# lpylpy0514/VitTracker

Hardware: AMD Instinct MI355X
Metric: track() frames/sec per GPU, vit_48_h32, 128px search / 64px template (higher is better)
Workload: dtype f32

## Files before the change

### vittracker_amd/csrc/vt_bf3.h

```cpp
#pragma once
#include "vt_common.h"

namespace vt3 {

typedef __bf16 bf16x8 __attribute__((ext_vector_type(8)));
typedef unsigned u32x2 __attribute__((ext_vector_type(2)));
typedef unsigned u32x4 __attribute__((ext_vector_type(4)));

#ifndef VT_SPLIT_DOT2
#define VT_SPLIT_DOT2 0
#endif
typedef __bf16 bf16x2 __attribute__((ext_vector_type(2)));
__device__ __forceinline__ void sub_pair(unsigned pair, float x0, float x1, float& r0, float& r1) {
    const bf16x2 a = __builtin_bit_cast(bf16x2, pair);
    unsigned sel_lo = 0x0000bf80u, sel_hi = 0xbf800000u;
    asm volatile("" : "+s"(sel_lo), "+s"(sel_hi));
    r0 = __builtin_amdgcn_fdot2_f32_bf16(a, __builtin_bit_cast(bf16x2, sel_lo), x0, false);
    r1 = __builtin_amdgcn_fdot2_f32_bf16(a, __builtin_bit_cast(bf16x2, sel_hi), x1, false);
}
__device__ __forceinline__ void split3(f4 x, u32x2& h, u32x2& m, u32x2& l) {
#ifdef VT_SPLIT_FAKE
    h = u32x2{__builtin_amdgcn_perm(__float_as_uint(x[1]), __float_as_uint(x[0]), 0x07060302u), __builtin_amdgcn_perm(__float_as_uint(x[3]), __float_as_uint(x[2]), 0x07060302u)};
    m = h; l = h;
    asm volatile("" : "+v"(m), "+v"(l));
    return;
#endif
#if VT_SPLIT_DOT2
#pragma unroll
    for (int p = 0; p < 2; ++p) {
        const float x0 = x[2 * p], x1 = x[2 * p + 1];
        float r0, r1, s0, s1;
        h[p] = __builtin_amdgcn_perm(__float_as_uint(x1), __float_as_uint(x0), 0x07060302u);
        sub_pair(h[p], x0, x1, r0, r1);
        m[p] = __builtin_amdgcn_perm(__float_as_uint(r1), __float_as_uint(r0), 0x07060302u);
        sub_pair(m[p], r0, r1, s0, s1);
        l[p] = __builtin_amdgcn_perm(__float_as_uint(s1), __float_as_uint(s0), 0x07060302u);
    }
#else
    unsigned xb[4], r1b[4], r2b[4];
#pragma unroll
    for (int i = 0; i < 4; ++i) {
        xb[i] = __float_as_uint(x[i]);
        const float r1 = x[i] - __uint_as_float(xb[i] & 0xffff0000u);
        r1b[i] = __float_as_uint(r1);
        const float r2 = r1 - __uint_as_float(r1b[i] & 0xffff0000u);
        r2b[i] = __float_as_uint(r2);
    }
    h = u32x2{__builtin_amdgcn_perm(xb[1], xb[0], 0x07060302u), __builtin_amdgcn_perm(xb[3], xb[2], 0x07060302u)};
    m = u32x2{__builtin_amdgcn_perm(r1b[1], r1b[0], 0x07060302u), __builtin_amdgcn_perm(r1b[3], r1b[2], 0x07060302u)};
    l = u32x2{__builtin_amdgcn_perm(r2b[1], r2b[0], 0x07060302u), __builtin_amdgcn_perm(r2b[3], r2b[2], 0x07060302u)};
#endif
}
__device__ __forceinline__ f4 join3(u32x2 h, u32x2 m, u32x2 l) {
    f4 v;
#pragma unroll
    for (int i = 0; i < 4; ++i) {
        const unsigned sh = (i & 1) ? 0u : 16u;
        const float fh = __uint_as_float((h[i >> 1] << sh) & 0xffff0000u), fm = __uint_as_float((m[i >> 1] << sh) & 0xffff0000u),
                    fl = __uint_as_float((l[i >> 1] << sh) & 0xffff0000u);
        v[i] = (fh + fm) + fl;
    }
    return v;
}

__device__ __forceinline__ f4 mma(u32x4 a, u32x4 b, f4 acc) {
    return __builtin_amdgcn_mfma_f32_16x16x32_bf16(__builtin_bit_cast(bf16x8, a), __builtin_bit_cast(bf16x8, b), acc, 0, 0, 0);
}
typedef short s16x4 __attribute__((ext_vector_type(4)));
__device__ __forceinline__ f4 mma16(u32x2 a, u32x2 b, f4 acc) {
    return __builtin_amdgcn_mfma_f32_16x16x16bf16_1k(__builtin_bit_cast(s16x4, a), __builtin_bit_cast(s16x4, b), acc, 0, 0, 0);
}
__device__ __forceinline__ f4 mma_small(const u32x4 (&a)[3], const u32x4 (&b)[3], f4 acc) {
    acc = mma(a[2], b[0], acc);
    acc = mma(a[0], b[2], acc);
    return mma(a[1], b[1], acc);
}
__device__ __forceinline__ f4 mma_large(const u32x4 (&a)[3], const u32x4 (&b)[3], f4 acc) {
    acc = mma(a[1], b[0], acc);
    acc = mma(a[0], b[1], acc);
    return mma(a[0], b[0], acc);
}

}
```

### vittracker_amd/csrc/vt_blocks.h

```cpp
#pragma once
#include <type_traits>
#include "vt_common.h"
#include "vt_bf3.h"

namespace vtb {

constexpr int C = 48;
constexpr int NC = C / 16;
constexpr int HID = 4 * C;
constexpr int NH = HID / 16;
constexpr float LN_EPS = 1e-5f;

constexpr int O_LN1G = 0;
constexpr int O_LN1B = O_LN1G + C;
constexpr int O_WQKV = O_LN1B + C;
constexpr int O_BQKV = O_WQKV + 9 * NC * 256;
constexpr int O_WPROJ = O_BQKV + 3 * C;
constexpr int O_BPROJ = O_WPROJ + NC * NC * 256;
constexpr int O_LN2G = O_BPROJ + C;
constexpr int O_LN2B = O_LN2G + C;
constexpr int O_W1 = O_LN2B + C;
constexpr int O_B1 = O_W1 + NH * NC * 256;
constexpr int O_W2 = O_B1 + HID;
constexpr int O_B2 = O_W2 + NC * NH * 256;
constexpr int BLOCK_STRIDE = O_B2 + C;
static_assert(BLOCK_STRIDE % 4 == 0 && O_WQKV % 4 == 0 && O_W1 % 4 == 0 && O_W2 % 4 == 0, "16B alignment");

constexpr int W3_FC1_TILES = NH * 3 + NH * 3 / 2;
constexpr int W3_FC1_OT16 = 3 * 64 + 3 * 32;
constexpr int W3_FC2_TILES = NC * (NH / 2) * 3;
constexpr int W3_QKV_TILES = (9 * W3_FC1_OT16 + 63) / 64;
constexpr int W3_PROJ_TILES = (NC * W3_FC1_OT16 + 63) / 64;
constexpr int BLOCK3_STRIDE = (W3_FC1_TILES + W3_FC2_TILES + W3_QKV_TILES + W3_PROJ_TILES) * 256;
static_assert(W3_FC1_TILES == 54 && W3_FC2_TILES == 54 && NH * W3_FC1_OT16 == W3_FC1_TILES * 64, "three-piece MLP images");

constexpr int S_LN1G = 0;
constexpr int S_LN1B = S_LN1G + C;
constexpr int S_BQKV = S_LN1B + C;
constexpr int S_BPROJ = S_BQKV + 3 * C;
constexpr int S_LN2G = S_BPROJ + C;
constexpr int S_LN2B = S_LN2G + C;
constexpr int S_B1 = S_LN2B + C;
constexpr int S_B2 = S_B1 + HID;
constexpr int SMALL_STRIDE = S_B2 + C;
static_assert(SMALL_STRIDE % 4 == 0 && S_BQKV % 4 == 0 && S_BPROJ % 4 == 0 && S_B1 % 4 == 0 && S_B2 % 4 == 0, "16B alignment");
static_assert(O_LN1B == O_LN1G + C && O_LN2G == O_BPROJ + C && O_LN2B == O_LN2G + C, "contiguous sections");
__host__ __device__ constexpr int small_floats(int depth) { return depth * SMALL_STRIDE + 2 * C; }

__device__ __forceinline__ size_t small_src(int f, int depth) {
    const int blk = f / SMALL_STRIDE, r = f - blk * SMALL_STRIDE;
    if (blk >= depth) return (size_t)depth * BLOCK_STRIDE + r;
    const int o = r < S_BQKV ? O_LN1G + r : r < S_BPROJ ? O_BQKV + (r - S_BQKV) : r < S_B1 ? O_BPROJ + (r - S_BPROJ)
                : r < S_B2 ? O_B1 + (r - S_B1) : O_B2 + (r - S_B2);
    return (size_t)blk * BLOCK_STRIDE + o;
}

__device__ __forceinline__ f4 wimg(const float* __restrict__ base, int tile, int lane) {
    return ld4(base + (size_t)tile * 256 + lane * 4);
}

__device__ __forceinline__ opnd wimg_o(const opnd* __restrict__ base, int tile, int lane) { return base[(size_t)tile * 64 + lane]; }

template <int N>
__device__ __forceinline__ void wburst(f4 (&a)[N], const float* __restrict__ base, int first, int stride, int lane) {
#pragma unroll
    for (int j = 0; j < N; ++j) a[j] = wimg(base, first + j * stride, lane);
    __builtin_amdgcn_sched_barrier(0);
}

template <int N, int VALU_PER_MFMA>
__device__ __forceinline__ void interleave_mfma_valu() {
#pragma unroll
    for (int n = 0; n < N; ++n) {
        __builtin_amdgcn_sched_group_barrier(0x008, 1, 0);
        __builtin_amdgcn_sched_group_barrier(0x002, VALU_PER_MFMA, 0);
    }
}

template <bool AFFINE = true>
__device__ __forceinline__ void layer_norm_img(const f4 (&x)[NC], f4 (&h)[NC], const float* __restrict__ g,
                                               const float* __restrict__ b, int q) {
    static_assert(NC == 3, "three feature chunks");
    const float mean = quad_sum(hsum4((x[0] + x[1]) + x[2])) * (1.0f / C);
    f4 d[NC];
#pragma unroll
    for (int c = 0; c < NC; ++c) d[c] = x[c] - splat4(mean);
    const f4 v4 = __builtin_elementwise_fma(d[2], d[2], __builtin_elementwise_fma(d[1], d[1], d[0] * d[0]));
    const float inv = __builtin_amdgcn_rsqf(quad_sum(hsum4(v4)) * (1.0f / C) + LN_EPS);
#pragma unroll
    for (int c = 0; c < NC; ++c) {
        if constexpr (AFFINE) {
            const f4 gg = ld4(g + 16 * c + 4 * q), bb = ld4(b + 16 * c + 4 * q);
            h[c] = d[c] * splat4(inv) * gg + bb;
        } else {
            h[c] = d[c] * splat4(inv);
        }
    }
}
__device__ __forceinline__ void layer_norm_plain(const f4 (&x)[NC], f4 (&h)[NC]) { layer_norm_img<false>(x, h, nullptr, nullptr, 0); }

constexpr int WBUF_TILES = NH * NC;
template <bool STAGED>
__device__ __forceinline__ void barrier_publish() {
    if constexpr (STAGED) asm volatile("s_waitcnt vmcnt(0)" ::: "memory");
    __syncthreads();
}

#ifndef VT_BLK_GUESTS
#define VT_BLK_GUESTS 1
#endif
#ifndef VT_BLK_OWNERS
#define VT_BLK_OWNERS 1
#endif
#ifndef VT_BLK_NOSTAGE
#define VT_BLK_NOSTAGE 0
#endif
__device__ __forceinline__ void stage_tiles(f4* dst, const float* __restrict__ src, int ntiles, int w, int nw, int lane, bool first_block = true) {
    if (VT_BLK_NOSTAGE == 1 || (VT_BLK_NOSTAGE == 2 && !first_block)) return;
    for (int t = w; t < ntiles; t += nw)
        __builtin_amdgcn_global_load_lds((const __attribute__((address_space(1))) void*)(src + (size_t)t * 256 + lane * 4),
                                         (__attribute__((address_space(3))) void*)(dst + t * 64), 16, 0, 0);
}

template <int NCHUNK, int N, bool SHARED_IS_B, bool PRELOAD_ALL = true, typename AT = opnd, typename OpA, typename OpS>
__device__ __forceinline__ void gemm_stage(OpA opa, OpS ops, f4 (&acc)[N]) {
    if constexpr (PRELOAD_ALL && NCHUNK * N <= 24) {
        AT a[NCHUNK][N];
#pragma unroll
        for (int c = 0; c < NCHUNK; ++c) opa(c, a[c]);
        __builtin_amdgcn_sched_barrier(0);
#pragma unroll
        for (int c = 0; c < NCHUNK; ++c) {
            if constexpr (SHARED_IS_B) mfma4_shared_b(a[c], ops(c), acc);
            else mfma4_shared_a(ops(c), a[c], acc);
        }
    } else {
        AT a[2][N];
        opa(0, a[0]);
#pragma unroll
        for (int c = 0; c < NCHUNK; ++c) {
            if (c + 1 < NCHUNK) opa(c + 1, a[(c + 1) & 1]);
            if constexpr (SHARED_IS_B) mfma4_shared_b(a[c & 1], ops(c), acc);
            else mfma4_shared_a(ops(c), a[c & 1], acc);
        }
    }
}

template <int NT, int NW, int TPW, bool WLDS, bool BAL = false, bool ZC = false, bool BF3 = false, bool A3 = false>
__global__ __launch_bounds__(NW * 64, (NW == 5 && !WLDS) ? 3 : 1) void blocks_kernel(const float* __restrict__ tokens,
                                                         const float* __restrict__ params,
                                                         float* __restrict__ feat,
                                                         float* __restrict__ resid,
                                                         int len_z, int depth_total, int nblocks,
                                                         int dbg_skip_tile,
                                                         unsigned long long* __restrict__ stamps,
                                                         float* __restrict__ zcache,
                                                         int zcache_mode,
                                                         const float* __restrict__ params3,
                                                         unsigned* __restrict__ vlscr) {
    static_assert(NW * TPW >= NT, "tiles must be covered");
    constexpr bool BF3L = BF3 && WLDS, BF3G = BF3 && !WLDS;
    static_assert(!BF3L || (BAL && 2 * NT * NC >= W3_FC2_TILES - WBUF_TILES), "BF3 with staging: written for the balanced frame form; fc2's third output tile is staged in the K / V area");
    static_assert(!BAL || (WLDS && TPW == 1 && NW == 2 * (NT - 1)), "balanced variant: NT-1 owners + NT-1 guests");
    static_assert(!A3 || BF3, "A3: written for the three-piece forms");
    constexpr bool VP3 = A3 && BF3L;
    constexpr bool VP2L = A3 && BF3G;
    constexpr int KP_T16 = W3_FC1_OT16, VP_PAIRS = NT / 2, VP_T16 = VP_PAIRS * 3 * 64 + (NT & 1) * 3 * 32;
    constexpr int KV_UNITS = A3 ? NT * KP_T16 + (VP3 ? NC * VP_T16 : NC * NT * 64) : 2 * NT * NC * 64;
    constexpr int L = NT * 16;
    constexpr int NOWN = BAL ? NT - 1 : NT;
    const int toff = (BAL && len_z == 16) ? 1 : 0;
    const int GT = toff ? 0 : NT - 1;
    extern __shared__ __attribute__((aligned(16))) float lds[];
    f4* Kimg = reinterpret_cast<f4*>(lds);
    f4* Vimg = Kimg + (A3 ? NT * KP_T16 : NT * NC * 64);
    opnd* const Ko = reinterpret_cast<opnd*>(Kimg);
    opnd* const Vo = reinterpret_cast<opnd*>(Vimg);
    f4* Wa = Kimg + KV_UNITS;
    constexpr int WA_TILES = BF3L ? W3_FC1_TILES : WBUF_TILES;
    f4* Wb = Wa + WA_TILES * 64;
    float* Sp = reinterpret_cast<float*>(WLDS ? Wb + WBUF_TILES * 64 : Wa);
    f4* const Gx = reinterpret_cast<f4*>(Sp + small_floats(depth_total));
    f4* Qg = A3 ? Wb + W3_PROJ_TILES * 64 : Gx;
    f4* Pg = Qg + (A3 ? KP_T16 : NC * 64);
    f4* Dg = A3 ? Gx : Pg + 4 * NC * 64;
    float* Mg = reinterpret_cast<float*>(A3 ? Pg + 4 * NC * 64 : Dg + NC * 64);
    int* gflag = A3 ? reinterpret_cast<int*>(Dg + NC * 64) : reinterpret_cast<int*>(Mg + 4 * 2 * 64);
    f4* Pg2 = A3 ? Wa + W3_QKV_TILES * 64 : Pg;
    static_assert(!A3 || (W3_PROJ_TILES * 64 + KP_T16 + 4 * NC * 64 + 4 * 2 * 64 / 4 <= WBUF_TILES * 64 && W3_QKV_TILES * 64 + 4 * NC * 64 <= W3_FC1_TILES * 64),
                  "A3: the exchange areas fit behind proj's / qkv's image");

    const int b = blockIdx.x;
    const int lane = threadIdx.x & 63;
    const int w = __builtin_amdgcn_readfirstlane(threadIdx.x >> 6);
    const int tok = lane & 15, q = lane >> 4;
    const int g = w - (NT - 1);
    const float scale = 0.14433756729740643f;
    constexpr float SCALE_LOG2E = 0.14433756729740643f * 1.4426950408889634f;
    const int guest_prio = dbg_skip_tile == -3 ? 0 : 1;
    const bool fine = dbg_skip_tile == -2 || dbg_skip_tile <= -100;
    if (dbg_skip_tile <= -100) dbg_skip_tile = -100 - dbg_skip_tile;
    int nstamp = 0;
    auto stamp = [&]() {
        if (stamps != nullptr) {
            unsigned long long t;
            asm volatile("s_memtime %0\n\ts_waitcnt lgkmcnt(0)" : "=s"(t)::"memory");
            if (lane == 0) stamps[((size_t)b * NW + w) * 64 + nstamp] = t;
            ++nstamp;
        }
    };
    auto fstamp = [&]() { if (fine) stamp(); };
    stamp();
    auto stage_img = [&](f4* dst, int off, int ntiles, int blk_of) {
        if constexpr (VT_IS_F16)
            stage_tiles(dst, reinterpret_cast<const float*>(reinterpret_cast<const _Float16*>(params3) + (size_t)blk_of * BLOCK_STRIDE + off), (ntiles + 1) / 2, w, NW, lane);
        else
            stage_tiles(dst, params + (size_t)blk_of * BLOCK_STRIDE + off, ntiles, w, NW, lane);
    };
    if constexpr (BF3L) stage_tiles(Wa, params3 + (W3_FC1_TILES + W3_FC2_TILES) * 256, W3_QKV_TILES, w, NW, lane);
    else if constexpr (WLDS) stage_img(Wa, O_WQKV, 9 * NC, 0);
    for (int i = threadIdx.x; 4 * i < small_floats(depth_total); i += NW * 64)
        st4(Sp + 4 * i, ld4(params + small_src(4 * i, depth_total)));

    f4 x[TPW][NC];
#pragma unroll
    for (int i = 0; i < TPW; ++i) {
        const int T = w + NW * i + toff;
        if (T - toff < NOWN && T != dbg_skip_tile) {
            const float* src = tokens + ((size_t)b * L + 16 * T + tok) * C + 4 * q;
#pragma unroll
            for (int c = 0; c < NC; ++c) x[i][c] = ld4(src + 16 * c);
        }
    }
    f4 x4s[NC];
    f4 (&x4)[NC] = (BAL && !BF3) ? x[0] : x4s;
    if constexpr (BAL) {
        if (w >= NOWN) {
            const float* src = tokens + ((size_t)b * L + 16 * GT + tok) * C + 4 * q;
#pragma unroll
            for (int c = 0; c < NC; ++c) x4[c] = ld4(src + 16 * c);
        }
        if (threadIdx.x == 0) *gflag = 0;
        if (w >= NOWN && guest_prio > 0) __builtin_amdgcn_s_setprio(2);
    }
    barrier_publish<WLDS>();

    const int lane_k = lane;
    for (int blk = 0; blk < nblocks; ++blk) {
        int lane_s = lane_k;
        if constexpr (BF3) asm volatile("" : "+v"(lane_s));
        const int lane = lane_s, tok = lane & 15, q = lane >> 4;
        const bool last_skip_z = (blk == depth_total - 1) && (resid == nullptr);
        const bool guest_skip = BAL && last_skip_z && toff != 0;
        const bool zg_tile = BAL && ZC && blk == 0 && toff != 0;
        const float* __restrict__ P = params + (size_t)blk * BLOCK_STRIDE;
        const float* S = Sp + blk * SMALL_STRIDE;
        const opnd* const Po = VT_IS_F16 ? reinterpret_cast<const opnd*>(reinterpret_cast<const _Float16*>(params3) + (size_t)blk * BLOCK_STRIDE)
                                         : reinterpret_cast<const opnd*>(P);
        const opnd* const Wa_o = reinterpret_cast<const opnd*>(Wa);
        const opnd* const Wb_o = reinterpret_cast<const opnd*>(Wb);
        auto w_qkv = [&](int t) { return WLDS ? Wa_o[t * 64 + lane] : wimg_o(Po + O_WQKV / 4, t, lane); };
        auto w_proj = [&](int t) { return WLDS ? Wb_o[t * 64 + lane] : wimg_o(Po + O_WPROJ / 4, t, lane); };
        auto w_fc1 = [&](int t) { return WLDS ? Wa_o[t * 64 + lane] : wimg_o(Po + O_W1 / 4, t, lane); };
        auto w_fc2 = [&](int t) { return WLDS ? Wb_o[t * 64 + lane] : wimg_o(Po + O_W2 / 4, t, lane); };
        const float* __restrict__ P3 = BF3 ? params3 + (size_t)blk * BLOCK3_STRIDE : nullptr;
        constexpr int PROJ_TILES = NC * NC;
        using vt3::u32x2;
        using vt3::u32x4;
        int lane3 = lane;
        if constexpr (BF3) asm volatile("" : "+v"(lane3));
        const auto Wa3 = BF3L ? lds_lane_base<u32x4>(Wa, 16u * lane3) : nullptr;
        const auto Wa3h = BF3L ? lds_lane_base<u32x2>(Wa, 192u * 16u + 8u * lane3) : nullptr;
        const auto Wb3 = BF3L ? lds_lane_base<u32x4>(Wb, 16u * lane3) : nullptr;
        const auto Wk3 = BF3L ? lds_lane_base<u32x4>(Kimg, 16u * lane3) : nullptr;
        auto w1_load3 = [&](int t, u32x4 (&a0)[3], u32x2 (&a2)[3]) {
#pragma unroll
            for (int pc = 0; pc < 3; ++pc) {
                a0[pc] = Wa3[t * W3_FC1_OT16 + pc * 64];
                a2[pc] = Wa3h[t * W3_FC1_OT16 * 2 + pc * 64];
            }
        };
        auto w2_load3 = [&](int p, u32x4 (&a)[NC][3]) {
#pragma unroll
            for (int ot = 0; ot < NC; ++ot)
#pragma unroll
                for (int pc = 0; pc < 3; ++pc)
                    a[ot][pc] = ot < 2 ? Wb3[((ot * (NH / 2) + p) * 3 + pc) * 64] : Wk3[(p * 3 + pc) * 64];
        };
        auto split_h3 = [&](const f4 (&h)[NC], u32x4 (&hb)[3], u32x2 (&hc)[3]) {
            u32x2 a[3], b2[3];
            vt3::split3(h[0], a[0], a[1], a[2]);
            vt3::split3(h[1], b2[0], b2[1], b2[2]);
            vt3::split3(h[2], hc[0], hc[1], hc[2]);
#pragma unroll
            for (int pc = 0; pc < 3; ++pc) hb[pc] = u32x4{a[pc].x, a[pc].y, b2[pc].x, b2[pc].y};
        };
        auto tile48 = [&](auto swap, const u32x4 (&a0)[3], const u32x2 (&a2)[3], const u32x4 (&hb)[3], const u32x2 (&hc)[3], f4 init) {
            constexpr bool SWAP = decltype(swap)::value;
            constexpr int TW[6] = {2, 0, 1, 1, 0, 0}, TX[6] = {0, 2, 1, 0, 1, 0};
            f4 accA = init, accB = splat4(0.f);
#pragma unroll
            for (int e = 0; e < 6; ++e) {
                accB = SWAP ? vt3::mma16(hc[TX[e]], a2[TW[e]], accB) : vt3::mma16(a2[TW[e]], hc[TX[e]], accB);
                accA = SWAP ? vt3::mma(hb[TX[e]], a0[TW[e]], accA) : vt3::mma(a0[TW[e]], hb[TX[e]], accA);
            }
            return accA + accB;
        };
        const auto Kp3 = A3 ? lds_lane_base<u32x4>(Kimg, 16u * lane3) : nullptr;
        const auto Kp3h = A3 ? lds_lane_base<u32x2>(Kimg, 192u * 16u + 8u * lane3) : nullptr;
        const auto Vp3 = A3 ? lds_lane_base<u32x4>(Kimg + NT * KP_T16, 16u * lane3) : nullptr;
        const auto Vp3h = A3 ? lds_lane_base<u32x2>(Kimg + NT * KP_T16, VP_PAIRS * 3 * 64 * 16u + 8u * lane3) : nullptr;
        auto k_load3 = [&](int J, u32x4 (&a0)[3], u32x2 (&a2)[3]) {
#pragma unroll
            for (int pc = 0; pc < 3; ++pc) {
                a0[pc] = Kp3[J * KP_T16 + pc * 64];
                a2[pc] = Kp3h[J * KP_T16 * 2 + pc * 64];
            }
        };
        auto wp_load3 = [&](int t, u32x4 (&a0)[3], u32x2 (&a2)[3]) {
            if constexpr (BF3L) {
#pragma unroll
                for (int pc = 0; pc < 3; ++pc) {
                    a0[pc] = Wb3[t * W3_FC1_OT16 + pc * 64];
                    a2[pc] = reinterpret_cast<const u32x2*>(Wb)[(t * W3_FC1_OT16 + 192) * 2 + pc * 64 + lane3];
                }
            } else {
                const u32x4* const Gp = reinterpret_cast<const u32x4*>(P3) + (W3_FC1_TILES + W3_FC2_TILES + W3_QKV_TILES) * 64;
#pragma unroll
                for (int pc = 0; pc < 3; ++pc) {
                    a0[pc] = Gp[t * W3_FC1_OT16 + pc * 64 + lane3];
                    a2[pc] = reinterpret_cast<const u32x2*>(Gp)[(t * W3_FC1_OT16 + 192) * 2 + pc * 64 + lane3];
                }
            }
        };
        auto store_k3 = [&](f4* dst_tile, const f4 (&kr)[NC]) {
            u32x4 kb[3];
            u32x2 kc[3];
            split_h3(kr, kb, kc);
#pragma unroll
            for (int pc = 0; pc < 3; ++pc) {
                reinterpret_cast<u32x4*>(dst_tile)[pc * 64 + lane3] = kb[pc];
                reinterpret_cast<u32x2*>(dst_tile + 192)[pc * 64 + lane3] = kc[pc];
            }
        };
        auto store_k3c = [&](f4* dst_tile, int ot, f4 r) {
            u32x2 pk[3];
            vt3::split3(r, pk[0], pk[1], pk[2]);
#pragma unroll
            for (int pc = 0; pc < 3; ++pc) {
                if (ot < 2) reinterpret_cast<u32x2*>(dst_tile)[(pc * 64 + lane3) * 2 + ot] = pk[pc];
                else reinterpret_cast<u32x2*>(dst_tile + 192)[pc * 64 + lane3] = pk[pc];
            }
        };
        auto store_v3 = [&](int T, int ot, f4 r) {
            u32x2 pv[3];
            vt3::split3(r, pv[0], pv[1], pv[2]);
            u32x2* base = reinterpret_cast<u32x2*>(Kimg + NT * KP_T16 + ot * VP_T16);
            if ((NT & 1) && T == NT - 1) {
#pragma unroll
                for (int pc = 0; pc < 3; ++pc) base[VP_PAIRS * 3 * 64 * 2 + pc * 64 + lane3] = pv[pc];
            } else {
#pragma unroll
                for (int pc = 0; pc < 3; ++pc) base[(((T >> 1) * 3 + pc) * 64 + lane3) * 2 + (T & 1)] = pv[pc];
            }
        };
        constexpr int VL_BLK_U4 = NC * VP_PAIRS * 64;
        u32x4* const vl_blk = VP2L ? reinterpret_cast<u32x4*>(vlscr) + ((size_t)b * depth_total + blk) * VL_BLK_U4 : nullptr;
        auto store_v2l = [&](int T, int ot, f4 r) {
            u32x2 pv[3];
            vt3::split3(r, pv[0], pv[1], pv[2]);
            const int pp = T >> 1, hf = T & 1;
#pragma unroll
            for (int pc = 0; pc < 2; ++pc) reinterpret_cast<u32x2*>(Vimg)[((((ot * VP_PAIRS + pp) * 2 + pc) * 64) + lane3) * 2 + hf] = pv[pc];
            reinterpret_cast<u32x2*>(vl_blk)[(((ot * VP_PAIRS + pp) * 64) + lane3) * 2 + hf] = pv[2];
        };
        if constexpr (A3 && BF3L) {
            stage_tiles(Wb, P3 + (W3_FC1_TILES + W3_FC2_TILES + W3_QKV_TILES) * 256, W3_PROJ_TILES, w, NW, lane, blk == 0);
        } else if constexpr (BF3L) {
            stage_tiles(Wb, P + O_WPROJ, PROJ_TILES, w, NW, lane, blk == 0);
        } else if constexpr (WLDS) stage_img(Wb, O_WPROJ, NC * NC, blk);

        f4 qr[TPW][NC];
#pragma unroll
        for (int i = 0; i < TPW; ++i) {
            const int T = w + NW * i + toff;
            const bool z_tile = ZC && blk == 0 && 16 * T < len_z;
            int lane_z = lane;
            if constexpr (ZC) asm volatile("" : "+v"(lane_z));
            f4* const zc = reinterpret_cast<f4*>(zcache) + (((size_t)b * (len_z >> 4) + T) * 3 * NC) * 64 + lane_z;
            if (VT_BLK_OWNERS && T - toff < NOWN && T != dbg_skip_tile && z_tile && zcache_mode == 2) {
#pragma unroll
                for (int ot = 0; ot < NC; ++ot) {
                    qr[i][ot] = zc[ot * 64];
                    if constexpr (VP3) store_v3(T, ot, zc[(2 * NC + ot) * 64]);
                    else if constexpr (VP2L) store_v2l(T, ot, zc[(2 * NC + ot) * 64]);
                    else Vo[(ot * NT + T) * 64 + lane] = to_opnd(zc[(2 * NC + ot) * 64]);
                    if constexpr (!A3) Ko[(T * NC + ot) * 64 + lane] = to_opnd(zc[(NC + ot) * 64]);
                }
                if constexpr (A3) {
                    f4 kr[NC];
#pragma unroll
                    for (int ot = 0; ot < NC; ++ot) kr[ot] = zc[(NC + ot) * 64];
                    store_k3(Kimg + T * KP_T16, kr);
                }
            } else if (VT_BLK_OWNERS && T - toff < NOWN && T != dbg_skip_tile) {
                f4 h[NC];
                layer_norm_plain(x[i], h);
                fstamp();
                if constexpr (BF3) {
                    u32x4 hb[3];
                    u32x2 hc[3];
                    split_h3(h, hb, hc);
                    const u32x4* const Gq = reinterpret_cast<const u32x4*>(P3) + (W3_FC1_TILES + W3_FC2_TILES) * 64;
                    const u32x2* const Gqh = reinterpret_cast<const u32x2*>(Gq);
                    auto wq_load3 = [&](int t, u32x4 (&a0)[3], u32x2 (&a2)[3]) {
                        if constexpr (BF3L) w1_load3(t, a0, a2);
                        else {
#pragma unroll
                            for (int pc = 0; pc < 3; ++pc) {
                                a0[pc] = Gq[t * W3_FC1_OT16 + pc * 64 + lane3];
                                a2[pc] = Gqh[(t * W3_FC1_OT16 + 192) * 2 + pc * 64 + lane3];
                            }
                        }
                    };
                    u32x4 a0[2][3];
                    u32x2 a2[2][3];
                    auto bias_q = [&](int t) { return t < 2 * NC ? ld4(S + S_BQKV + 16 * t + 4 * q) : splat4(S[S_BQKV + 2 * C + 16 * (t % NC) + tok]); };
                    f4 bias[2];
                    f4 kr[NC];
                    wq_load3(0, a0[0], a2[0]);
                    bias[0] = bias_q(0);
#pragma unroll
                    for (int t = 0; t < 3 * NC; ++t) {
                        if (t + 1 < 3 * NC) {
                            wq_load3(t + 1, a0[(t + 1) & 1], a2[(t + 1) & 1]);
                            bias[(t + 1) & 1] = bias_q(t + 1);
                        }
                        const int ot = t % NC;
                        f4 r;
                        __builtin_amdgcn_sched_barrier(0);
                        if (t < 2 * NC) r = tile48(std::false_type{}, a0[t & 1], a2[t & 1], hb, hc, bias[t & 1]);
                        else r = tile48(std::true_type{}, a0[t & 1], a2[t & 1], hb, hc, bias[t & 1]);
                        if (t < NC) qr[i][ot] = r;
                        else if constexpr (A3) {
                            if (t < 2 * NC) {
                                if constexpr (VP3) {
                                    kr[ot] = r;
                                    if (ot == NC - 1) store_k3(Kimg + T * KP_T16, kr);
                                } else store_k3c(Kimg + T * KP_T16, ot, r);
                            } else if constexpr (VP3) store_v3(T, ot, r);
                            else if constexpr (VP2L) store_v2l(T, ot, r);
                            else Vo[(ot * NT + T) * 64 + lane] = to_opnd(r);
                        }
                        else if (t < 2 * NC) Ko[(T * NC + ot) * 64 + lane] = to_opnd(r);
                        else Vo[(ot * NT + T) * 64 + lane] = to_opnd(r);
                        if (z_tile && zcache_mode == 1) zc[t * 64] = r;
                        if (t == 2 * NC - 1) fstamp();
                    }
                } else {
                {
                    f4 acc[2 * NC];
#pragma unroll
                    for (int ot = 0; ot < 2 * NC; ++ot) acc[ot] = ld4(S + S_BQKV + 16 * ot + 4 * q);
                    gemm_stage<NC, 2 * NC, true, WLDS>(
                        [&](int c, opnd (&a)[2 * NC]) {
#pragma unroll
                            for (int ot = 0; ot < 2 * NC; ++ot) a[ot] = w_qkv(ot * NC + c);
                        },
                        [&](int c) { return h[c]; }, acc);
#pragma unroll
                    for (int ot = 0; ot < NC; ++ot) {
                        qr[i][ot] = acc[ot];
                        Ko[(T * NC + ot) * 64 + lane] = to_opnd(acc[NC + ot]);
                        if (z_tile && zcache_mode == 1) { zc[ot * 64] = acc[ot]; zc[(NC + ot) * 64] = acc[NC + ot]; }
                    }
                }
                fstamp();
                {
                    f4 acc[NC];
#pragma unroll
                    for (int ot = 0; ot < NC; ++ot) acc[ot] = splat4(S[S_BQKV + 2 * C + 16 * ot + tok]);
                    gemm_stage<NC, NC, false, WLDS>(
                        [&](int c, opnd (&bw)[NC]) {
#pragma unroll
                            for (int ot = 0; ot < NC; ++ot) bw[ot] = w_qkv((2 * NC + ot) * NC + c);
                        },
                        [&](int c) { return h[c]; }, acc);
#pragma unroll
                    for (int ot = 0; ot < NC; ++ot) {
                        Vo[(ot * NT + T) * 64 + lane] = to_opnd(acc[ot]);
                        if (z_tile && zcache_mode == 1) zc[(2 * NC + ot) * 64] = acc[ot];
                    }
                }
                }
            }
        }
        if constexpr (BAL) {
            auto zc_guest = [&]() {
                int lane_z = lane;
                asm volatile("" : "+v"(lane_z));
                return reinterpret_cast<f4*>(zcache) + ((size_t)b * 3 * NC + NC * g) * 64 + lane_z;
            };
            auto with_gt = [&](auto f) {
                if (toff) f(std::integral_constant<int, 0>{});
                else f(std::integral_constant<int, NT - 1>{});
            };
            const bool guest_qkv = VT_BLK_GUESTS && w >= NOWN && g < 3 && !(guest_skip && g == 0);
            if (BF3L && guest_qkv) {
                f4 r[NC];
                if (zg_tile && zcache_mode == 2) {
                    const f4* const zc = zc_guest();
#pragma unroll
                    for (int j = 0; j < NC; ++j) r[j] = zc[j * 64];
                } else {
                    f4 h[NC];
                    layer_norm_plain(x4, h);
                    u32x4 hb[3];
                    u32x2 hc[3];
                    split_h3(h, hb, hc);
                    u32x4 a0[NC][3];
                    u32x2 a2[NC][3];
#pragma unroll
                    for (int j = 0; j < NC; ++j) w1_load3(NC * g + j, a0[j], a2[j]);
                    if (g < 2) {
                        f4 bias[NC];
#pragma unroll
                        for (int j = 0; j < NC; ++j) bias[j] = ld4(S + S_BQKV + 16 * (g * NC + j) + 4 * q);
                        __builtin_amdgcn_sched_barrier(0);
#pragma unroll
                        for (int j = 0; j < NC; ++j) r[j] = tile48(std::false_type{}, a0[j], a2[j], hb, hc, bias[j]);
                    } else {
                        f4 bias[NC];
#pragma unroll
                        for (int j = 0; j < NC; ++j) bias[j] = splat4(S[S_BQKV + 2 * C + 16 * j + tok]);
                        __builtin_amdgcn_sched_barrier(0);
#pragma unroll
                        for (int j = 0; j < NC; ++j) r[j] = tile48(std::true_type{}, a0[j], a2[j], hb, hc, bias[j]);
                    }
                    if (zg_tile && zcache_mode == 1) {
                        f4* const zc = zc_guest();
#pragma unroll
                        for (int j = 0; j < NC; ++j) zc[j * 64] = r[j];
                    }
                }
                with_gt([&](auto gt) {
                    constexpr int GTc = decltype(gt)::value;
                    if (g < 2) {
                        if constexpr (A3) {
                            store_k3(g == 0 ? Qg : Kimg + GTc * KP_T16, r);
                        } else {
#pragma unroll
                            for (int j = 0; j < NC; ++j) {
                                if (g == 0) Qg[j * 64 + lane] = r[j];
                                else Ko[(GTc * NC + j) * 64 + lane] = to_opnd(r[j]);
                            }
                        }
                    } else {
#pragma unroll
                        for (int j = 0; j < NC; ++j) {
                            if constexpr (A3) store_v3(GTc, j, r[j]);
                            else Vo[(j * NT + GTc) * 64 + lane] = to_opnd(r[j]);
                        }
                    }
                });
            } else if (guest_qkv) {
                f4 acc[NC];
                if (zg_tile && zcache_mode == 2) {
                    const f4* const zc = zc_guest();
#pragma unroll
                    for (int ot = 0; ot < NC; ++ot) acc[ot] = zc[ot * 64];
                } else {
                    f4 h[NC];
                    layer_norm_plain(x4, h);
                    if (g < 2) {
#pragma unroll
                        for (int ot = 0; ot < NC; ++ot) acc[ot] = ld4(S + S_BQKV + 16 * (g * NC + ot) + 4 * q);
                        gemm_stage<NC, NC, true, true>(
                            [&](int c, opnd (&a)[NC]) {
#pragma unroll
                                for (int ot = 0; ot < NC; ++ot) a[ot] = w_qkv((g * NC + ot) * NC + c);
                            },
                            [&](int c) { return h[c]; }, acc);
                    } else {
#pragma unroll
                        for (int ot = 0; ot < NC; ++ot) acc[ot] = splat4(S[S_BQKV + 2 * C + 16 * ot + tok]);
                        gemm_stage<NC, NC, false, true>(
                            [&](int c, opnd (&bw)[NC]) {
#pragma unroll
                                for (int ot = 0; ot < NC; ++ot) bw[ot] = w_qkv((2 * NC + ot) * NC + c);
                            },
                            [&](int c) { return h[c]; }, acc);
                    }
                    if (zg_tile && zcache_mode == 1) {
                        f4* const zc = zc_guest();
#pragma unroll
                        for (int ot = 0; ot < NC; ++ot) zc[ot * 64] = acc[ot];
                    }
                }
                with_gt([&](auto gt) {
                    constexpr int GTc = decltype(gt)::value;
#pragma unroll
                    for (int ot = 0; ot < NC; ++ot) {
                        if (g == 0) Qg[ot * 64 + lane] = acc[ot];
                        else if (g == 1) Ko[(GTc * NC + ot) * 64 + lane] = to_opnd(acc[ot]);
                        else Vo[(ot * NT + GTc) * 64 + lane] = to_opnd(acc[ot]);
                    }
                });
            }
        }
        stamp();
        if constexpr (VP2L) asm volatile("s_waitcnt vmcnt(0)" ::: "memory");
        barrier_publish<WLDS>();
        stamp();
        if constexpr (BF3L) {
            stage_tiles(Wa, P3, W3_FC1_TILES, w, NW, lane, blk == 0);
        } else if constexpr (WLDS) stage_img(Wa, O_W1, NH * NC, blk);
#pragma unroll
        for (int i = 0; i < TPW; ++i) {
            const int T = w + NW * i + toff;
            if (A3 && VT_BLK_OWNERS && T - toff < NOWN && T != dbg_skip_tile && !(last_skip_z && 16 * T < len_z)) {
                constexpr int TW[6] = {2, 0, 1, 1, 0, 0}, TX[6] = {0, 2, 1, 0, 1, 0};
                u32x4 qb[3];
                u32x2 qc[3];
                split_h3(qr[i], qb, qc);
                f4 s[NT];
                float m0 = -3.0e38f, m1 = -3.0e38f;
                {
                    constexpr int NB = VP3 ? 2 : 1;
                    u32x4 a0[NB][3];
                    u32x2 a2[NB][3];
                    if (NB == 2) k_load3(0, a0[0], a2[0]);
#pragma unroll
                    for (int J = 0; J < NT; ++J) {
                        if (NB == 2 && J + 1 < NT) k_load3(J + 1, a0[(J + 1) % NB], a2[(J + 1) % NB]);
                        if (NB == 1) k_load3(J, a0[0], a2[0]);
                        __builtin_amdgcn_sched_barrier(0);
                        s[J] = tile48(std::false_type{}, a0[J % NB], a2[J % NB], qb, qc, splat4(0.f));
                        m0 = fmaxf(fmaxf(m0, s[J].x), s[J].y);
                        m1 = fmaxf(fmaxf(m1, s[J].z), s[J].w);
                    }
                }
                fstamp();
                const float m = quad_max(fmaxf(m0, m1));
                const f2 k2 = {SCALE_LOG2E, SCALE_LOG2E}, nm2 = {-m * SCALE_LOG2E, -m * SCALE_LOG2E};
                f2 d0 = {0.f, 0.f}, d1 = {0.f, 0.f};
                f4 o[NC];
                constexpr int NWB = VP3 ? 2 : 1;
                u32x4 wa0[NWB][3];
                u32x2 wa2[NWB][3];
                if constexpr (VP3) {
                    u32x4 pb[VP_PAIRS > 0 ? VP_PAIRS : 1][3];
                    u32x2 po[3], plo[3];
                    u32x4 v[NC][3];
                    auto v_load3 = [&](int pp) {
#pragma unroll
                        for (int t = 0; t < NC; ++t)
#pragma unroll
                            for (int pc = 0; pc < 3; ++pc) v[t][pc] = Vp3[t * VP_T16 + (pp * 3 + pc) * 64];
                    };
                    if (VP_PAIRS > 0) v_load3(0);
#pragma unroll
                    for (int J = 0; J < NT; ++J) {
                        const f2 a = __builtin_elementwise_fma(f2{s[J].x, s[J].y}, k2, nm2);
                        const f2 c = __builtin_elementwise_fma(f2{s[J].z, s[J].w}, k2, nm2);
                        const f2 ea = {__builtin_amdgcn_exp2f(a.x), __builtin_amdgcn_exp2f(a.y)};
                        const f2 ec = {__builtin_amdgcn_exp2f(c.x), __builtin_amdgcn_exp2f(c.y)};
                        d0 += ea;
                        d1 += ec;
                        u32x2 pj[3];
                        vt3::split3(f4{ea.x, ea.y, ec.x, ec.y}, pj[0], pj[1], pj[2]);
#pragma unroll
                        for (int pc = 0; pc < 3; ++pc) {
                            if ((NT & 1) && J == NT - 1) po[pc] = pj[pc];
                            else if (J & 1) pb[J >> 1][pc] = u32x4{plo[pc].x, plo[pc].y, pj[pc].x, pj[pc].y};
                            else plo[pc] = pj[pc];
                        }
                    }
                    const f2 dd = d0 + d1;
                    const float rden = __builtin_amdgcn_rcpf(quad_sum(dd.x + dd.y));
                    fstamp();
                    f4 oA[NC], oB[NC];
#pragma unroll
                    for (int t = 0; t < NC; ++t) oA[t] = oB[t] = splat4(0.f);
                    u32x2 vh[NC][3];
                    if (NT & 1) {
#pragma unroll
                        for (int t = 0; t < NC; ++t)
#pragma unroll
                            for (int pc = 0; pc < 3; ++pc) vh[t][pc] = Vp3h[t * VP_T16 * 2 + pc * 64];
                    }
#pragma unroll
                    for (int pp = 0; pp < VP_PAIRS; ++pp) {
                        __builtin_amdgcn_sched_barrier(0);
#pragma unroll
                        for (int e = 0; e < 6; ++e)
#pragma unroll
                            for (int t = 0; t < NC; ++t) oA[t] = vt3::mma(v[t][TW[e]], pb[pp][TX[e]], oA[t]);
                        __builtin_amdgcn_sched_barrier(0);
                        if (pp + 1 < VP_PAIRS) v_load3(pp + 1);
                    }
                    wp_load3(0, wa0[0], wa2[0]);
                    if (NT & 1) {
                        __builtin_amdgcn_sched_barrier(0);
#pragma unroll
                        for (int e = 0; e < 6; ++e)
#pragma unroll
                            for (int t = 0; t < NC; ++t) oB[t] = vt3::mma16(vh[t][TW[e]], po[TX[e]], oB[t]);
                    }
#pragma unroll
                    for (int t = 0; t < NC; ++t) o[t] = (oA[t] + oB[t]) * splat4(rden);
                } else if constexpr (VP2L) {
                    const auto Vp2 = lds_lane_base<u32x4>(Vimg, 16u * lane3);
                    const u32x4* const vlg = vl_blk + lane3;
                    u32x4 vl[2][NC];
#pragma unroll
                    for (int t = 0; t < NC; ++t) vl[0][t] = vlg[(t * VP_PAIRS) * 64];
                    f4 oA[NC];
#pragma unroll
                    for (int t = 0; t < NC; ++t) oA[t] = splat4(0.f);
#pragma unroll
                    for (int pp = 0; pp < VP_PAIRS; ++pp) {
                        if (pp + 1 < VP_PAIRS) {
#pragma unroll
                            for (int t = 0; t < NC; ++t) vl[(pp + 1) & 1][t] = vlg[(t * VP_PAIRS + pp + 1) * 64];
                        }
                        u32x4 v[NC][2];
#pragma unroll
                        for (int t = 0; t < NC; ++t)
#pragma unroll
                            for (int pc = 0; pc < 2; ++pc) v[t][pc] = Vp2[((t * VP_PAIRS + pp) * 2 + pc) * 64];
                        u32x2 pj[2][3];
#pragma unroll
                        for (int jj = 0; jj < 2; ++jj) {
                            const int J = 2 * pp + jj;
                            const f2 a = __builtin_elementwise_fma(f2{s[J].x, s[J].y}, k2, nm2);
                            const f2 c = __builtin_elementwise_fma(f2{s[J].z, s[J].w}, k2, nm2);
                            const f2 ea = {__builtin_amdgcn_exp2f(a.x), __builtin_amdgcn_exp2f(a.y)};
                            const f2 ec = {__builtin_amdgcn_exp2f(c.x), __builtin_amdgcn_exp2f(c.y)};
                            d0 += ea;
                            d1 += ec;
                            vt3::split3(f4{ea.x, ea.y, ec.x, ec.y}, pj[jj][0], pj[jj][1], pj[jj][2]);
                        }
                        u32x4 pb[3];
#pragma unroll
                        for (int pc = 0; pc < 3; ++pc) pb[pc] = u32x4{pj[0][pc].x, pj[0][pc].y, pj[1][pc].x, pj[1][pc].y};
                        __builtin_amdgcn_sched_barrier(0);
#pragma unroll
                        for (int e = 0; e < 6; ++e)
#pragma unroll
                            for (int t = 0; t < NC; ++t) oA[t] = vt3::mma(TW[e] == 2 ? vl[pp & 1][t] : v[t][TW[e] & 1], pb[TX[e]], oA[t]);
                        __builtin_amdgcn_sched_barrier(0);
                    }
                    const f2 dd = d0 + d1;
                    const float rden = __builtin_amdgcn_rcpf(quad_sum(dd.x + dd.y));
                    fstamp();
#pragma unroll
                    for (int t = 0; t < NC; ++t) o[t] = oA[t] * splat4(rden);
                } else {
#pragma unroll
                    for (int J = 0; J < NT; ++J) {
                        const f2 a = __builtin_elementwise_fma(f2{s[J].x, s[J].y}, k2, nm2);
                        const f2 c = __builtin_elementwise_fma(f2{s[J].z, s[J].w}, k2, nm2);
                        const f2 ea = {__builtin_amdgcn_exp2f(a.x), __builtin_amdgcn_exp2f(a.y)};
                        const f2 ec = {__builtin_amdgcn_exp2f(c.x), __builtin_amdgcn_exp2f(c.y)};
                        s[J] = f4{ea.x, ea.y, ec.x, ec.y};
                        d0 += ea;
                        d1 += ec;
                    }
                    const f2 dd = d0 + d1;
                    const float rden = __builtin_amdgcn_rcpf(quad_sum(dd.x + dd.y));
                    fstamp();
#pragma unroll
                    for (int t = 0; t < NC; ++t) o[t] = splat4(0.f);
                    gemm_stage<NT, NC, true, WLDS>(
                        [&](int J, opnd (&a)[NC]) {
#pragma unroll
                            for (int t = 0; t < NC; ++t) a[t] = Vo[(t * NT + J) * 64 + lane];
                        },
                        [&](int J) { return s[J]; }, o);
#pragma unroll
                    for (int t = 0; t < NC; ++t) o[t] = o[t] * splat4(rden);
                }
                fstamp();
                u32x4 ob[3];
                u32x2 oc[3];
                split_h3(o, ob, oc);
#pragma unroll
                for (int ot = 0; ot < NC; ++ot) {
                    if (NWB == 2 && ot + 1 < NC) wp_load3(ot + 1, wa0[(ot + 1) % NWB], wa2[(ot + 1) % NWB]);
                    if (NWB == 1) wp_load3(ot, wa0[0], wa2[0]);
                    __builtin_amdgcn_sched_barrier(0);
                    x[i][ot] = tile48(std::false_type{}, wa0[ot % NWB], wa2[ot % NWB], ob, oc, x[i][ot] + ld4(S + S_BPROJ + 16 * ot + 4 * q));
                    __builtin_amdgcn_sched_barrier(0);
                }
            } else if (!A3 && VT_BLK_OWNERS && T - toff < NOWN && T != dbg_skip_tile && !(last_skip_z && 16 * T < len_z)) {
                f4 s[NT];
                float m0 = -3.0e38f, m1 = -3.0e38f;
                constexpr int JG = 5;
                static_assert(NT % JG == 0, "NT must be a multiple of 5");
#pragma unroll
                for (int j0 = 0; j0 < NT; j0 += JG) {
                    f4 acc[JG];
#pragma unroll
                    for (int j = 0; j < JG; ++j) acc[j] = splat4(0.f);
                    gemm_stage<NC, JG, true, WLDS>(
                        [&](int c, opnd (&a)[JG]) {
#pragma unroll
                            for (int j = 0; j < JG; ++j) a[j] = Ko[((j0 + j) * NC + c) * 64 + lane];
                        },
                        [&](int c) { return qr[i][c]; }, acc);
#pragma unroll
                    for (int j = 0; j < JG; ++j) {
                        s[j0 + j] = acc[j];
                        m0 = fmaxf(fmaxf(m0, acc[j].x), acc[j].y);
                        m1 = fmaxf(fmaxf(m1, acc[j].z), acc[j].w);
                    }
                }
                fstamp();
                const float m = quad_max(fmaxf(m0, m1));
                const f2 k2 = {SCALE_LOG2E, SCALE_LOG2E}, nm2 = {-m * SCALE_LOG2E, -m * SCALE_LOG2E};
                f2 d0 = {0.f, 0.f}, d1 = {0.f, 0.f};
#pragma unroll
                for (int J = 0; J < NT; ++J) {
                    const f2 a = __builtin_elementwise_fma(f2{s[J].x, s[J].y}, k2, nm2);
                    const f2 c = __builtin_elementwise_fma(f2{s[J].z, s[J].w}, k2, nm2);
                    const f2 ea = {__builtin_amdgcn_exp2f(a.x), __builtin_amdgcn_exp2f(a.y)};
                    const f2 ec = {__builtin_amdgcn_exp2f(c.x), __builtin_amdgcn_exp2f(c.y)};
                    s[J] = f4{ea.x, ea.y, ec.x, ec.y};
                    d0 += ea;
                    d1 += ec;
                }
                const f2 dd = d0 + d1;
                const float den = dd.x + dd.y;
                const float rden = __builtin_amdgcn_rcpf(quad_sum(den));
                fstamp();
                f4 o[NC];
#pragma unroll
                for (int t = 0; t < NC; ++t) o[t] = splat4(0.f);
                gemm_stage<NT, NC, true, WLDS>(
                    [&](int J, opnd (&a)[NC]) {
#pragma unroll
                        for (int t = 0; t < NC; ++t) a[t] = Vo[(t * NT + J) * 64 + lane];
                    },
                    [&](int J) { return s[J]; }, o);
#pragma unroll
                for (int t = 0; t < NC; ++t) o[t] = o[t] * splat4(rden);
                fstamp();
#pragma unroll
                for (int ot = 0; ot < NC; ++ot) x[i][ot] = x[i][ot] + ld4(S + S_BPROJ + 16 * ot + 4 * q);
                gemm_stage<NC, NC, true, WLDS>(
                    [&](int c, opnd (&a)[NC]) {
#pragma unroll
                        for (int ot = 0; ot < NC; ++ot) a[ot] = w_proj(ot * NC + c);
                    },
                    [&](int c) { return o[c]; }, x[i]);
            }
        }
        if constexpr (BAL) {
            if (VT_BLK_GUESTS && w >= NOWN && !guest_skip) {
                auto attn_part = [&](auto njc, int J0) {
                    constexpr int NJ = decltype(njc)::value;
                    f4 qv[NC];
#pragma unroll
                    for (int c = 0; c < NC; ++c) qv[c] = Qg[c * 64 + lane];
                    f4 sc[NJ];
#pragma unroll
                    for (int j = 0; j < NJ; ++j) sc[j] = splat4(0.f);
                    gemm_stage<NC, NJ, true, true>(
                        [&](int c, opnd (&a)[NJ]) {
#pragma unroll
                            for (int j = 0; j < NJ; ++j) a[j] = Ko[((J0 + j) * NC + c) * 64 + lane];
                        },
                        [&](int c) { return qv[c]; }, sc);
                    float m0 = -3.0e38f, m1 = -3.0e38f;
#pragma unroll
                    for (int j = 0; j < NJ; ++j) {
                        m0 = fmaxf(fmaxf(m0, sc[j].x), sc[j].y);
                        m1 = fmaxf(fmaxf(m1, sc[j].z), sc[j].w);
                    }
                    const float mraw = quad_max(fmaxf(m0, m1));
                    const float m = mraw * scale;
                    const f2 k2 = {SCALE_LOG2E, SCALE_LOG2E}, nm2 = {-mraw * SCALE_LOG2E, -mraw * SCALE_LOG2E};
                    f2 d0 = {0.f, 0.f}, d1 = {0.f, 0.f};
#pragma unroll
                    for (int j = 0; j < NJ; ++j) {
                        const f2 a = __builtin_elementwise_fma(f2{sc[j].x, sc[j].y}, k2, nm2);
                        const f2 c = __builtin_elementwise_fma(f2{sc[j].z, sc[j].w}, k2, nm2);
                        const f2 ea = {__builtin_amdgcn_exp2f(a.x), __builtin_amdgcn_exp2f(a.y)};
                        const f2 ec = {__builtin_amdgcn_exp2f(c.x), __builtin_amdgcn_exp2f(c.y)};
                        sc[j] = f4{ea.x, ea.y, ec.x, ec.y};
                        d0 += ea;
                        d1 += ec;
                    }
                    const f2 dd = d0 + d1;
                    float den = dd.x + dd.y;
                    den = quad_sum(den);
                    f4 o[NC];
#pragma unroll
                    for (int t = 0; t < NC; ++t) o[t] = splat4(0.f);
                    gemm_stage<NJ, NC, true, true>(
                        [&](int J, opnd (&a)[NC]) {
#pragma unroll
                            for (int t = 0; t < NC; ++t) a[t] = Vo[(t * NT + J0 + J) * 64 + lane];
                        },
                        [&](int J) { return sc[J]; }, o);
#pragma unroll
                    for (int t = 0; t < NC; ++t) Pg[(g * NC + t) * 64 + lane] = o[t];
                    Mg[(g * 2 + 0) * 64 + lane] = m;
                    Mg[(g * 2 + 1) * 64 + lane] = den;
                };
                auto attn_part3 = [&](auto njc, int J0) {
                    constexpr int NJ = decltype(njc)::value;
                    constexpr int TW[6] = {2, 0, 1, 1, 0, 0}, TX[6] = {0, 2, 1, 0, 1, 0};
                    u32x4 qb[3];
                    u32x2 qc[3];
                    u32x4 a0[NJ][3];
                    u32x2 a2[NJ][3];
#pragma unroll
                    for (int pc = 0; pc < 3; ++pc) {
                        qb[pc] = reinterpret_cast<const u32x4*>(Qg)[pc * 64 + lane3];
                        qc[pc] = reinterpret_cast<const u32x2*>(Qg + 192)[pc * 64 + lane3];
                    }
#pragma unroll
                    for (int j = 0; j < NJ; ++j) k_load3(J0 + j, a0[j], a2[j]);
                    u32x2 vh[NJ][NC][3];
#pragma unroll
                    for (int j = 0; j < NJ; ++j) {
                        const int J = J0 + j;
                        const bool oddc = (NT & 1) && J == NT - 1;
#pragma unroll
                        for (int t = 0; t < NC; ++t) {
                            const u32x2* base = reinterpret_cast<const u32x2*>(Kimg + NT * KP_T16 + t * VP_T16);
#pragma unroll
                            for (int pc = 0; pc < 3; ++pc)
                                vh[j][t][pc] = oddc ? base[VP_PAIRS * 3 * 64 * 2 + pc * 64 + lane3] : base[(((J >> 1) * 3 + pc) * 64 + lane3) * 2 + (J & 1)];
                        }
                    }
                    __builtin_amdgcn_sched_barrier(0);
                    f4 sc[NJ];
#pragma unroll
                    for (int j = 0; j < NJ; ++j) sc[j] = tile48(std::false_type{}, a0[j], a2[j], qb, qc, splat4(0.f));
                    float m0 = -3.0e38f, m1 = -3.0e38f;
#pragma unroll
                    for (int j = 0; j < NJ; ++j) {
                        m0 = fmaxf(fmaxf(m0, sc[j].x), sc[j].y);
                        m1 = fmaxf(fmaxf(m1, sc[j].z), sc[j].w);
                    }
                    const float mraw = quad_max(fmaxf(m0, m1));
                    const float m = mraw * scale;
                    const f2 k2 = {SCALE_LOG2E, SCALE_LOG2E}, nm2 = {-mraw * SCALE_LOG2E, -mraw * SCALE_LOG2E};
                    f2 d0 = {0.f, 0.f}, d1 = {0.f, 0.f};
                    u32x2 pp[NJ][3];
#pragma unroll
                    for (int j = 0; j < NJ; ++j) {
                        const f2 a = __builtin_elementwise_fma(f2{sc[j].x, sc[j].y}, k2, nm2);
                        const f2 c = __builtin_elementwise_fma(f2{sc[j].z, sc[j].w}, k2, nm2);
                        const f2 ea = {__builtin_amdgcn_exp2f(a.x), __builtin_amdgcn_exp2f(a.y)};
                        const f2 ec = {__builtin_amdgcn_exp2f(c.x), __builtin_amdgcn_exp2f(c.y)};
                        d0 += ea;
                        d1 += ec;
                        vt3::split3(f4{ea.x, ea.y, ec.x, ec.y}, pp[j][0], pp[j][1], pp[j][2]);
                    }
                    const f2 dd = d0 + d1;
                    const float den = quad_sum(dd.x + dd.y);
                    f4 o[NC];
#pragma unroll
                    for (int t = 0; t < NC; ++t) o[t] = splat4(0.f);
#pragma unroll
                    for (int j = 0; j < NJ; ++j)
#pragma unroll
                        for (int e = 0; e < 6; ++e)
#pragma unroll
                            for (int t = 0; t < NC; ++t) o[t] = vt3::mma16(vh[j][t][TW[e]], pp[j][TX[e]], o[t]);
#pragma unroll
                    for (int t = 0; t < NC; ++t) Pg[(g * NC + t) * 64 + lane] = o[t];
                    Mg[(g * 2 + 0) * 64 + lane] = m;
                    Mg[(g * 2 + 1) * 64 + lane] = den;
                };
                if constexpr (A3) {
                    if (g == 3) attn_part3(std::integral_constant<int, NT - 3>{}, 3);
                    else attn_part3(std::integral_constant<int, 1>{}, g);
                } else {
                    if (g == 3) attn_part(std::integral_constant<int, NT - 3>{}, 3);
                    else attn_part(std::integral_constant<int, 1>{}, g);
                }
                __builtin_amdgcn_fence(__ATOMIC_RELEASE, "workgroup");
                if (lane == 0) __hip_atomic_fetch_add(gflag, 1, __ATOMIC_RELAXED, __HIP_MEMORY_SCOPE_WORKGROUP);
                if (g < 3) {
                    while (__hip_atomic_load(gflag, __ATOMIC_RELAXED, __HIP_MEMORY_SCOPE_WORKGROUP) < 4 * (blk + 1))
                        __builtin_amdgcn_s_sleep(1);
                    __builtin_amdgcn_fence(__ATOMIC_ACQUIRE, "workgroup");
                    float mk[4], lk[4], M = -3.0e38f;
#pragma unroll
                    for (int k = 0; k < 4; ++k) {
                        mk[k] = Mg[(k * 2 + 0) * 64 + lane];
                        lk[k] = Mg[(k * 2 + 1) * 64 + lane];
                        M = fmaxf(M, mk[k]);
                    }
                    float Lsum = 0.f;
                    f4 o[NC];
#pragma unroll
                    for (int t = 0; t < NC; ++t) o[t] = splat4(0.f);
#pragma unroll
                    for (int k = 0; k < 4; ++k) {
                        const float f = __expf(mk[k] - M);
                        Lsum = fmaf(f, lk[k], Lsum);
#pragma unroll
                        for (int t = 0; t < NC; ++t) o[t] = o[t] + splat4(f) * Pg[(k * NC + t) * 64 + lane];
                    }
                    const float rl = __builtin_amdgcn_rcpf(Lsum);
#pragma unroll
                    for (int t = 0; t < NC; ++t) o[t] = o[t] * splat4(rl);
                    if constexpr (A3) {
                        u32x4 ob[3], wa0[3];
                        u32x2 oc[3], wa2[3];
                        wp_load3(g, wa0, wa2);
                        split_h3(o, ob, oc);
                        Dg[g * 64 + lane] = tile48(std::false_type{}, wa0, wa2, ob, oc, splat4(0.f));
                    } else {
                        f4 acc[1] = {splat4(0.f)};
                        gemm_stage<NC, 1, true, true>([&](int c, opnd (&a)[1]) { a[0] = w_proj(g * NC + c); },
                                                      [&](int c) { return o[c]; }, acc);
                        Dg[g * 64 + lane] = acc[0];
                    }
                }
            }
        }
        stamp();
        barrier_publish<WLDS>();
        stamp();
        if constexpr (BF3L) {
            stage_tiles(Wb, P3 + W3_FC1_TILES * 256, WBUF_TILES, w, NW, lane, blk == 0);
            stage_tiles(Kimg, P3 + (W3_FC1_TILES + WBUF_TILES) * 256, W3_FC2_TILES - WBUF_TILES, w, NW, lane, blk == 0);
        } else if constexpr (WLDS) stage_img(Wb, O_W2, NC * NH, blk);
        constexpr int HG = 4;
        static_assert(NH / HG == 3, "pipeline written for 12 hidden tiles");
        constexpr int NHID = WLDS ? TPW : 1;
        f4 hid[NHID][NH];
        f4 acc2[NHID][HG];
        auto fc1 = [&](const f4 (&h)[NC], int g, f4 (&acc)[HG]) {
#pragma unroll
            for (int j = 0; j < HG; ++j) acc[j] = ld4(S + S_B1 + 16 * (HG * g + j) + 4 * q);
            gemm_stage<NC, HG, true, WLDS>(
                [&](int c, opnd (&a)[HG]) {
#pragma unroll
                    for (int j = 0; j < HG; ++j) a[j] = w_fc1((HG * g + j) * NC + c);
                },
                [&](int c) { return h[c]; }, acc);
        };
        auto gelu_group = [&](const f4 (&acc)[HG], f4 (&hd)[NH], int g) {
#pragma unroll
            for (int j = 0; j < HG; ++j)
                hd[HG * g + j] = gelu4(acc[j]);
        };
        auto fc2 = [&](const f4 (&hd)[NH], int g, f4 (&xo)[NC]) {
            gemm_stage<HG, NC, true, WLDS>(
                [&](int cc, opnd (&a)[NC]) {
#pragma unroll
                    for (int ot = 0; ot < NC; ++ot) a[ot] = w_fc2(ot * NH + HG * g + cc);
                },
                [&](int cc) { return hd[HG * g + cc]; }, xo);
        };
        auto mlp_first = [&](int i, int hi) {
            f4 h[NC];
            layer_norm_plain(x[i], h);
#pragma unroll
            for (int ot = 0; ot < NC; ++ot) x[i][ot] = x[i][ot] + ld4(S + S_B2 + 16 * ot + 4 * q);
            f4 acc0[HG], acc1[HG];
            fstamp();
            fc1(h, 0, acc0);
            __builtin_amdgcn_sched_barrier(0);
            fstamp();
            fc1(h, 1, acc1);
            gelu_group(acc0, hid[hi], 0);
            interleave_mfma_valu<12 * HG, 3>();
            __builtin_amdgcn_sched_barrier(0);
            fstamp();
            fc1(h, 2, acc2[hi]);
            gelu_group(acc1, hid[hi], 1);
            interleave_mfma_valu<12 * HG, 3>();
            __builtin_amdgcn_sched_barrier(0);
        };
        auto mlp_second = [&](int i, int hi) {
            fc2(hid[hi], 0, x[i]);
            gelu_group(acc2[hi], hid[hi], 2);
            interleave_mfma_valu<12 * HG, 3>();
            __builtin_amdgcn_sched_barrier(0);
            fstamp();
            fc2(hid[hi], 1, x[i]);
            fstamp();
            fc2(hid[hi], 2, x[i]);
        };
        auto fc1_terms3 = [&](auto nc, const u32x4 (*a0)[3], const u32x2 (*a2)[3], const u32x4 (&hb)[3], const u32x2 (&hc)[3], f4* acc) {
            constexpr int N = decltype(nc)::value;
            constexpr int TW[6] = {2, 0, 1, 1, 0, 0}, TX[6] = {0, 2, 1, 0, 1, 0};
            f4 accB[N];
#pragma unroll
            for (int j = 0; j < N; ++j) accB[j] = splat4(0.f);
#pragma unroll
            for (int half = 0; half < 2; ++half)
#pragma unroll
                for (int k = 0; k < 2; ++k)
#pragma unroll
                    for (int t3 = 0; t3 < 3; ++t3)
#pragma unroll
                        for (int j = 0; j < N; ++j) {
                            const int e = 3 * half + t3;
                            if (k == 0) accB[j] = vt3::mma16(a2[j][TW[e]], hc[TX[e]], accB[j]);
                            else acc[j] = vt3::mma(a0[j][TW[e]], hb[TX[e]], acc[j]);
                        }
#pragma unroll
            for (int j = 0; j < N; ++j) acc[j] = acc[j] + accB[j];
        };
        u32x4 hq[NHID][NH / 2][3];
        auto mlp_first3 = [&](int i, int hi) {
            f4 h[NC];
            layer_norm_plain(x[i], h);
#pragma unroll
            for (int ot = 0; ot < NC; ++ot) x[i][ot] = x[i][ot] + ld4(S + S_B2 + 16 * ot + 4 * q);
            u32x4 hb[3];
            u32x2 hc[3];
            split_h3(h, hb, hc);
            fstamp();
            constexpr int TW[6] = {2, 0, 1, 1, 0, 0}, TX[6] = {0, 2, 1, 0, 1, 0};
            u32x4 a0[2][3];
            u32x2 a2[2][3];
            w1_load3(0, a0[0], a2[0]);
            f4 bias1[2];
            bias1[0] = ld4(S + S_B1 + 4 * q);
            f4 prev = splat4(0.f);
            u32x2 pl[3];
            f2 ua, ub, na, nb, pa, pb, ea, eb;
            unsigned xb[4], r1b[4], r2b[4];
            [[maybe_unused]] u32x2 hpk, mpk;
            auto gstage = [&](int e) {
                const auto fma2 = [](f2 p, f2 n, float c) { return __builtin_elementwise_fma(p, n, f2{c, c}); };
                if (e == 0) {
                    ua = f2{prev.x, prev.y}; ub = f2{prev.z, prev.w};
                    na = f2{__builtin_fmaxf(-__builtin_fabsf(ua.x), -6.5f), __builtin_fmaxf(-__builtin_fabsf(ua.y), -6.5f)};
                    nb = f2{__builtin_fmaxf(-__builtin_fabsf(ub.x), -6.5f), __builtin_fmaxf(-__builtin_fabsf(ub.y), -6.5f)};
                    pa = __builtin_elementwise_fma(na, f2{2.992413958e-05f, 2.992413958e-05f}, f2{7.398738213e-04f, 7.398738213e-04f});
                    pb = __builtin_elementwise_fma(nb, f2{2.992413958e-05f, 2.992413958e-05f}, f2{7.398738213e-04f, 7.398738213e-04f});
                    pa = fma2(pa, na, 7.977461502e-03f); pb = fma2(pb, nb, 7.977461502e-03f);
                } else if (e == 1) {
                    pa = fma2(pa, na, 5.323818492e-02f); pb = fma2(pb, nb, 5.323818492e-02f);
                    pa = fma2(pa, na, -4.589156874e-01f); pb = fma2(pb, nb, -4.589156874e-01f);
                    pa = fma2(pa, na, 1.151147082e+00f); pb = fma2(pb, nb, 1.151147082e+00f);
                    pa = fma2(pa, na, -1.0f); pb = fma2(pb, nb, -1.0f);
                } else if (e == 2) {
                    ea = f2{__builtin_amdgcn_exp2f(pa.x), __builtin_amdgcn_exp2f(pa.y)};
                    eb = f2{__builtin_amdgcn_exp2f(pb.x), __builtin_amdgcn_exp2f(pb.y)};
                    ua = f2{fmaxf(ua.x, 0.0f), fmaxf(ua.y, 0.0f)};
                    ub = f2{fmaxf(ub.x, 0.0f), fmaxf(ub.y, 0.0f)};
                } else if (e == 3) {
                    const f2 ga = __builtin_elementwise_fma(na, ea, ua), gb = __builtin_elementwise_fma(nb, eb, ub);
                    const float gv[4] = {ga.x, ga.y, gb.x, gb.y};
#if VT_SPLIT_DOT2
#pragma unroll
                    for (int p2 = 0; p2 < 2; ++p2) {
                        float r0, r1;
                        hpk[p2] = __builtin_amdgcn_perm(__float_as_uint(gv[2 * p2 + 1]), __float_as_uint(gv[2 * p2]), 0x07060302u);
                        vt3::sub_pair(hpk[p2], gv[2 * p2], gv[2 * p2 + 1], r0, r1);
                        r1b[2 * p2] = __float_as_uint(r0); r1b[2 * p2 + 1] = __float_as_uint(r1);
                    }
#else
#pragma unroll
                    for (int k = 0; k < 4; ++k) {
                        xb[k] = __float_as_uint(gv[k]);
                        r1b[k] = __float_as_uint(gv[k] - __uint_as_float(xb[k] & 0xffff0000u));
                    }
#endif
                } else if (e == 4) {
#if VT_SPLIT_DOT2
#pragma unroll
                    for (int p2 = 0; p2 < 2; ++p2) {
                        float r0, r1;
                        mpk[p2] = __builtin_amdgcn_perm(r1b[2 * p2 + 1], r1b[2 * p2], 0x07060302u);
                        vt3::sub_pair(mpk[p2], __uint_as_float(r1b[2 * p2]), __uint_as_float(r1b[2 * p2 + 1]), r0, r1);
                        r2b[2 * p2] = __float_as_uint(r0); r2b[2 * p2 + 1] = __float_as_uint(r1);
                    }
#else
#pragma unroll
                    for (int k = 0; k < 4; ++k) r2b[k] = __float_as_uint(__uint_as_float(r1b[k]) - __uint_as_float(r1b[k] & 0xffff0000u));
#endif
                }
            };
            auto gfinish = [&](int t) {
                u32x2 pc3[3];
#if VT_SPLIT_DOT2
                pc3[0] = hpk;
                pc3[1] = mpk;
#else
                pc3[0] = u32x2{__builtin_amdgcn_perm(xb[1], xb[0], 0x07060302u), __builtin_amdgcn_perm(xb[3], xb[2], 0x07060302u)};
                pc3[1] = u32x2{__builtin_amdgcn_perm(r1b[1], r1b[0], 0x07060302u), __builtin_amdgcn_perm(r1b[3], r1b[2], 0x07060302u)};
#endif
                pc3[2] = u32x2{__builtin_amdgcn_perm(r2b[1], r2b[0], 0x07060302u), __builtin_amdgcn_perm(r2b[3], r2b[2], 0x07060302u)};
#pragma unroll
                for (int pc = 0; pc < 3; ++pc) asm volatile("" : "+v"(pc3[pc]));
                if (t & 1) {
#pragma unroll
                    for (int pc = 0; pc < 3; ++pc) hq[hi][t >> 1][pc] = u32x4{pl[pc].x, pl[pc].y, pc3[pc].x, pc3[pc].y};
                } else {
#pragma unroll
                    for (int pc = 0; pc < 3; ++pc) pl[pc] = pc3[pc];
                }
            };
#pragma unroll
            for (int t = 0; t <= NH; ++t) {
                if (t == 4 || t == 8) fstamp();
                f4 accA = splat4(0.f), accB = splat4(0.f);
                if (t < NH) {
                    accA = bias1[t & 1];
                    if (t + 1 < NH) {
                        w1_load3(t + 1, a0[(t + 1) & 1], a2[(t + 1) & 1]);
                        bias1[(t + 1) & 1] = ld4(S + S_B1 + 16 * (t + 1) + 4 * q);
                    }
                }
                __builtin_amdgcn_sched_barrier(0);
#pragma unroll
                for (int e = 0; e < 6; ++e) {
                    if (t < NH) {
                        accB = vt3::mma16(a2[t & 1][TW[e]], hc[TX[e]], accB);
                        accA = vt3::mma(a0[t & 1][TW[e]], hb[TX[e]], accA);
                    }
                    if (t > 0) {
                        if (e < 5) gstage(e);
                        else gfinish(t - 1);
                    }
                    __builtin_amdgcn_sched_barrier(0);
                }
                prev = accA + accB;
            }
        };
        auto mlp_second3 = [&](int i, int hi) {
            constexpr int NP = NH / 2;
            constexpr int TW[6] = {2, 0, 1, 1, 0, 0}, TX[6] = {0, 2, 1, 0, 1, 0};
            u32x4 a[2][NC][3];
            w2_load3(0, a[0]);
#pragma unroll
            for (int p = 0; p < NP; ++p) {
                if (p + 1 < NP) w2_load3(p + 1, a[(p + 1) & 1]);
                __builtin_amdgcn_sched_barrier(0);
#pragma unroll
                for (int e = 0; e < 6; ++e)
#pragma unroll
                    for (int ot = 0; ot < NC; ++ot) x[i][ot] = vt3::mma(a[p & 1][ot][TW[e]], hq[hi][p][TX[e]], x[i][ot]);
                if (p == 1 || p == 3) fstamp();
            }
        };
        if constexpr (BF3L) {
#pragma unroll
            for (int i = 0; i < TPW; ++i) {
                const int T = w + NW * i + toff;
                if (VT_BLK_OWNERS && T - toff < NOWN && T != dbg_skip_tile && !(last_skip_z && 16 * T < len_z)) mlp_first3(i, i);
            }
            u32x2 gq[NC][3];
            if (VT_BLK_GUESTS && w >= NOWN && !guest_skip) {
#pragma unroll
                for (int ot = 0; ot < NC; ++ot) x4[ot] = x4[ot] + ld4(S + S_BPROJ + 16 * ot + 4 * q) + Dg[ot * 64 + lane];
                f4 h[NC];
                layer_norm_plain(x4, h);
#pragma unroll
                for (int ot = 0; ot < NC; ++ot) x4[ot] = x4[ot] + ld4(S + S_B2 + 16 * ot + 4 * q);
                u32x4 hb[3];
                u32x2 hc[3];
                split_h3(h, hb, hc);
                u32x4 a0[NC][3];
                u32x2 a2[NC][3];
#pragma unroll
                for (int j = 0; j < NC; ++j) w1_load3(NC * g + j, a0[j], a2[j]);
                f4 acc[NC];
#pragma unroll
                for (int j = 0; j < NC; ++j) acc[j] = ld4(S + S_B1 + 16 * (NC * g + j) + 4 * q);
                __builtin_amdgcn_sched_barrier(0);
                fc1_terms3(std::integral_constant<int, NC>{}, a0, a2, hb, hc, acc);
#pragma unroll
                for (int j = 0; j < NC; ++j) vt3::split3(gelu4(acc[j]), gq[j][0], gq[j][1], gq[j][2]);
            }
                stamp();
            barrier_publish<true>();
            if (blk + 1 < nblocks) stage_tiles(Wa, P3 + BLOCK3_STRIDE + (W3_FC1_TILES + W3_FC2_TILES) * 256, W3_QKV_TILES, w, NW, lane, false);
            stamp();
#pragma unroll
            for (int i = 0; i < TPW; ++i) {
                const int T = w + NW * i + toff;
                if (VT_BLK_OWNERS && T - toff < NOWN && T != dbg_skip_tile && !(last_skip_z && 16 * T < len_z)) mlp_second3(i, i);
            }
            if (VT_BLK_GUESTS && w >= NOWN && !guest_skip) {
                const bool odd = g & 1;
                const int p_full = (3 * g + (odd ? 1 : 0)) >> 1, p_half = (3 * g + (odd ? 0 : 2)) >> 1;
                u32x4 bf[3];
                u32x2 bh[3];
#pragma unroll
                for (int pc = 0; pc < 3; ++pc) {
                    bf[pc] = odd ? u32x4{gq[1][pc].x, gq[1][pc].y, gq[2][pc].x, gq[2][pc].y} : u32x4{gq[0][pc].x, gq[0][pc].y, gq[1][pc].x, gq[1][pc].y};
                    bh[pc] = odd ? gq[0][pc] : gq[2][pc];
                }
                u32x4 af[NC][3];
                u32x2 ah[NC][3];
                w2_load3(p_full, af);
                {
                    const unsigned hoff = 16u * lane3 + (odd ? 8u : 0u) + (unsigned)p_half * (3u * 64u * 16u);
                    const auto Wb3h = lds_lane_base<u32x2>(Wb, hoff);
                    const auto Wk3h = lds_lane_base<u32x2>(Kimg, hoff);
#pragma unroll
                    for (int ot = 0; ot < NC; ++ot)
#pragma unroll
                        for (int pc = 0; pc < 3; ++pc)
                            ah[ot][pc] = ot < 2 ? Wb3h[((ot * (NH / 2)) * 3 + pc) * 64 * 2] : Wk3h[pc * 64 * 2];
                }
                f4 part[NC], partB[NC];
#pragma unroll
                for (int ot = 0; ot < NC; ++ot) part[ot] = partB[ot] = splat4(0.f);
                __builtin_amdgcn_sched_barrier(0);
                constexpr int TW[6] = {2, 0, 1, 1, 0, 0}, TX[6] = {0, 2, 1, 0, 1, 0};
#pragma unroll
                for (int half = 0; half < 2; ++half)
#pragma unroll
                    for (int k = 0; k < 2; ++k)
#pragma unroll
                        for (int t3 = 0; t3 < 3; ++t3)
#pragma unroll
                            for (int ot = 0; ot < NC; ++ot) {
                                const int e = 3 * half + t3;
                                if (k == 0) partB[ot] = vt3::mma16(ah[ot][TW[e]], bh[TX[e]], partB[ot]);
                                else part[ot] = vt3::mma(af[ot][TW[e]], bf[TX[e]], part[ot]);
                            }
#pragma unroll
                for (int ot = 0; ot < NC; ++ot) part[ot] = part[ot] + partB[ot];
#pragma unroll
                for (int ot = 0; ot < NC; ++ot) Pg2[(g * NC + ot) * 64 + lane] = part[ot];
            }
        } else if constexpr (WLDS) {
#pragma unroll
            for (int i = 0; i < TPW; ++i) {
                const int T = w + NW * i + toff;
                if (VT_BLK_OWNERS && T - toff < NOWN && T != dbg_skip_tile && !(last_skip_z && 16 * T < len_z)) mlp_first(i, i);
            }
            f4 ghid[NC];
            if constexpr (BAL) {
                if (VT_BLK_GUESTS && w >= NOWN && !guest_skip) {
#pragma unroll
                    for (int ot = 0; ot < NC; ++ot) x4[ot] = x4[ot] + ld4(S + S_BPROJ + 16 * ot + 4 * q) + Dg[ot * 64 + lane];
                    f4 h[NC];
                    layer_norm_plain(x4, h);
#pragma unroll
                    for (int ot = 0; ot < NC; ++ot) x4[ot] = x4[ot] + ld4(S + S_B2 + 16 * ot + 4 * q);
#pragma unroll
                    for (int j = 0; j < NC; ++j) ghid[j] = ld4(S + S_B1 + 16 * (NC * g + j) + 4 * q);
                    gemm_stage<NC, NC, true, true>(
                        [&](int c, opnd (&a)[NC]) {
#pragma unroll
                            for (int j = 0; j < NC; ++j) a[j] = w_fc1((NC * g + j) * NC + c);
                        },
                        [&](int c) { return h[c]; }, ghid);
#pragma unroll
                    for (int j = 0; j < NC; ++j)
                        ghid[j] = gelu4(ghid[j]);
                }
            }
            stamp();
            barrier_publish<WLDS>();
            if (blk + 1 < nblocks) stage_img(Wa, O_WQKV, 9 * NC, blk + 1);
            stamp();
#pragma unroll
            for (int i = 0; i < TPW; ++i) {
                const int T = w + NW * i + toff;
                if (VT_BLK_OWNERS && T - toff < NOWN && T != dbg_skip_tile && !(last_skip_z && 16 * T < len_z)) mlp_second(i, i);
            }
            if constexpr (BAL) {
                if (VT_BLK_GUESTS && w >= NOWN && !guest_skip) {
                    f4 part[NC];
#pragma unroll
                    for (int ot = 0; ot < NC; ++ot) part[ot] = splat4(0.f);
                    gemm_stage<NC, NC, true, true>(
                        [&](int cc, opnd (&a)[NC]) {
#pragma unroll
                            for (int ot = 0; ot < NC; ++ot) a[ot] = w_fc2(ot * NH + NC * g + cc);
                        },
                        [&](int cc) { return ghid[cc]; }, part);
#pragma unroll
                    for (int ot = 0; ot < NC; ++ot) Pg[(g * NC + ot) * 64 + lane] = part[ot];
                }
            }
        } else {
#pragma unroll
            for (int i = 0; i < TPW; ++i) {
                const int T = w + NW * i;
                if (BF3G && T < NT && T != dbg_skip_tile && !(last_skip_z && 16 * T < len_z)) {
                    const u32x4* const G1 = reinterpret_cast<const u32x4*>(P3);
                    const u32x2* const G1h = reinterpret_cast<const u32x2*>(P3);
                    const u32x4* const G2 = G1 + W3_FC1_TILES * 64;
                    auto g1_load3 = [&](int t, u32x4 (&a0)[3], u32x2 (&a2)[3]) {
#pragma unroll
                        for (int pc = 0; pc < 3; ++pc) {
                            a0[pc] = G1[t * W3_FC1_OT16 + pc * 64 + lane3];
                            a2[pc] = G1h[(t * W3_FC1_OT16 + 192) * 2 + pc * 64 + lane3];
                        }
                    };
                    f4 h[NC];
                    layer_norm_plain(x[i], h);
                    u32x4 hb[3];
                    u32x2 hc[3];
                    split_h3(h, hb, hc);
                    u32x4 hq3[NH / 2][3];
                    {
                        u32x4 a0[2][3];
                        u32x2 a2[2][3];
                        g1_load3(0, a0[0], a2[0]);
                        u32x2 pl[3];
#pragma unroll
                        for (int t = 0; t < NH; ++t) {
                            if (t + 1 < NH) g1_load3(t + 1, a0[(t + 1) & 1], a2[(t + 1) & 1]);
                            const f4 bias = ld4(S + S_B1 + 16 * t + 4 * q);
                            __builtin_amdgcn_sched_barrier(0);
                            const f4 r = tile48(std::false_type{}, a0[t & 1], a2[t & 1], hb, hc, bias);
                            u32x2 pc3[3];
                            vt3::split3(gelu4(r), pc3[0], pc3[1], pc3[2]);
#pragma unroll
                            for (int pc = 0; pc < 3; ++pc) {
                                if (t & 1) hq3[t >> 1][pc] = u32x4{pl[pc].x, pl[pc].y, pc3[pc].x, pc3[pc].y};
                                else pl[pc] = pc3[pc];
                            }
                        }
                    }
#pragma unroll
                    for (int ot = 0; ot < NC; ++ot) x[i][ot] = x[i][ot] + ld4(S + S_B2 + 16 * ot + 4 * q);
                    {
                        constexpr int NP = NH / 2;
                        constexpr int TW[6] = {2, 0, 1, 1, 0, 0}, TX[6] = {0, 2, 1, 0, 1, 0};
                        auto g2_load3 = [&](int st, u32x4 (&a)[3]) {
                            const int p = st / NC, ot = st - NC * p;
#pragma unroll
                            for (int pc = 0; pc < 3; ++pc) a[pc] = G2[((ot * NP + p) * 3 + pc) * 64 + lane3];
                        };
                        constexpr int NS = NP * NC, AHEAD = 3;
                        u32x4 a[AHEAD + 1][3];
#pragma unroll
                        for (int st = 0; st < AHEAD; ++st) g2_load3(st, a[st]);
#pragma unroll
                        for (int st = 0; st < NS; ++st) {
                            if (st + AHEAD < NS) g2_load3(st + AHEAD, a[(st + AHEAD) % (AHEAD + 1)]);
                            __builtin_amdgcn_sched_barrier(0);
                            const int p = st / NC, ot = st - NC * p;
#pragma unroll
                            for (int e = 0; e < 6; ++e) x[i][ot] = vt3::mma(a[st % (AHEAD + 1)][TW[e]], hq3[p][TX[e]], x[i][ot]);
                        }
                    }
                } else if (T < NT && T != dbg_skip_tile && !(last_skip_z && 16 * T < len_z)) {
                    f4 h[NC];
                    layer_norm_plain(x[i], h);
                    f4 hd[NH];
                    constexpr int G6 = 6;
#pragma unroll
                    for (int g = 0; g < NH; g += G6) {
                        f4 acc[G6];
#pragma unroll
                        for (int j = 0; j < G6; ++j) acc[j] = ld4(S + S_B1 + 16 * (g + j) + 4 * q);
#pragma unroll
                        for (int c = 0; c < NC; ++c) {
                            opnd a[G6];
#pragma unroll
                            for (int j = 0; j < G6; ++j) a[j] = w_fc1((g + j) * NC + c);
                            mfma4_shared_b(a, h[c], acc);
                        }
#pragma unroll
                        for (int j = 0; j < G6; ++j)
                            hd[g + j] = gelu4(acc[j]);
                    }
#pragma unroll
                    for (int ot = 0; ot < NC; ++ot) x[i][ot] = x[i][ot] + ld4(S + S_B2 + 16 * ot + 4 * q);
#pragma unroll
                    for (int c = 0; c < NH; ++c) {
                        opnd a[NC];
#pragma unroll
                        for (int ot = 0; ot < NC; ++ot) a[ot] = w_fc2(ot * NH + c);
                        mfma4_shared_b(a, hd[c], x[i]);
                    }
                }
            }
        }
        stamp();
        if constexpr (WLDS) barrier_publish<true>();
        if constexpr (BAL) {
            if (w >= NOWN && !guest_skip) {
#pragma unroll
                for (int k = 0; k < 4; ++k)
#pragma unroll
                    for (int ot = 0; ot < NC; ++ot) x4[ot] = x4[ot] + Pg2[(k * NC + ot) * 64 + lane];
            }
        }
    }

    stamp();
    const float* PF = Sp + depth_total * SMALL_STRIDE;
    int lane_e = lane_k;
    if constexpr (BF3) asm volatile("" : "+v"(lane_e));
    const int tok_e = lane_e & 15, q_e = lane_e >> 4;
    const int Lx = L - len_z;
    if constexpr (BAL) {
        if (g == 0) {
            if (resid != nullptr) {
                float* dst = resid + ((size_t)b * L + 16 * GT + tok_e) * C + 4 * q_e;
#pragma unroll
                for (int c = 0; c < NC; ++c) st4(dst + 16 * c, x4[c]);
            }
            if (16 * GT >= len_z) {
                f4 h[NC];
                layer_norm_img(x4, h, PF, PF + C, q_e);
                float* dst = feat + ((size_t)b * Lx + (16 * GT - len_z) + tok_e) * C + 4 * q_e;
#pragma unroll
                for (int c = 0; c < NC; ++c) st4(dst + 16 * c, h[c]);
            }
        }
    }
#pragma unroll
    for (int i = 0; i < TPW; ++i) {
        const int T = w + NW * i + toff;
        if (T - toff < NOWN) {
            if (resid != nullptr) {
                float* dst = resid + ((size_t)b * L + 16 * T + tok_e) * C + 4 * q_e;
#pragma unroll
                for (int c = 0; c < NC; ++c) st4(dst + 16 * c, x[i][c]);
            }
            if (16 * T >= len_z) {
                f4 h[NC];
                layer_norm_img(x[i], h, PF, PF + C, q_e);
                float* dst = feat + ((size_t)b * Lx + (16 * T - len_z) + tok_e) * C + 4 * q_e;
#pragma unroll
                for (int c = 0; c < NC; ++c) st4(dst + 16 * c, h[c]);
            }
        }
    }
}

}
```

Before: 3.256 million.

## Fold odd-K bf16 three-piece products into 16x16x32 MFMAs instead of 16x16x16

In the LDS-staged three-piece bf16 path, the six odd-half products that used 16x16x16 MFMAs into a separate accumulator are packed pairwise into three 16x16x32 MFMAs accumulating directly into the main accumulator. Operands are concatenated (hi|mid, hi|lo weight pairs; lo|hi, hi|mid, mid|hi activations) and weight halves are loaded through duplicated LDS base pointers. This halves the small MFMA count and removes the second accumulator and final add, at the cost of extra register packing and a changed summation order. It also simplifies K storage for VP3 and aliases x4 for BF3.

```diff
diff --git a/vittracker_amd/csrc/vt_bf3.h b/vittracker_amd/csrc/vt_bf3.h
--- a/vittracker_amd/csrc/vt_bf3.h
+++ b/vittracker_amd/csrc/vt_bf3.h
@@ -66,6 +66,32 @@
 __device__ __forceinline__ f4 mma(u32x4 a, u32x4 b, f4 acc) {
     return __builtin_amdgcn_mfma_f32_16x16x32_bf16(__builtin_bit_cast(bf16x8, a), __builtin_bit_cast(bf16x8, b), acc, 0, 0, 0);
 }
+struct odd_w { u32x4 hm, hl; };
+struct odd_x { u32x4 lh, hm, mh; };
+__device__ __forceinline__ u32x4 cat2(u32x2 a, u32x2 b) { return u32x4{a.x, a.y, b.x, b.y}; }
+__device__ __forceinline__ odd_w make_odd_w(const u32x2 (&w)[3]) { return odd_w{cat2(w[0], w[1]), cat2(w[0], w[2])}; }
+__device__ __forceinline__ odd_x make_odd_x(const u32x2 (&x)[3]) { return odd_x{cat2(x[2], x[0]), cat2(x[0], x[1]), cat2(x[1], x[0])}; }
+__device__ __forceinline__ odd_w ld_odd_w(lds_cptr<u32x2> p, lds_cptr<u32x2> p2, int idx, int stride = 64) {
+    odd_w r;
+    r.hm = cat2(p2[idx], p2[idx + stride]);
+    r.hl = cat2(p[idx], p[idx + 2 * stride]);
+    return r;
+}
+template <int STEP, bool SWAP = false>
+__device__ __forceinline__ f4 mma_odd(const odd_w& w, const odd_x& x, f4 acc) {
+    static_assert(STEP >= 0 && STEP < 3, "three steps");
+    const u32x4 ww = STEP == 0 ? w.hl : w.hm;
+    const u32x4 xw = STEP == 0 ? x.lh : STEP == 1 ? x.mh : x.hm;
+    return SWAP ? mma(xw, ww, acc) : mma(ww, xw, acc);
+}
+template <bool SWAP = false>
+__device__ __forceinline__ f4 mma_odd3(const u32x2 (&w)[3], const u32x2 (&x)[3], f4 acc) {
+    const odd_w wr = make_odd_w(w);
+    const odd_x xr = make_odd_x(x);
+    acc = mma_odd<0, SWAP>(wr, xr, acc);
+    acc = mma_odd<1, SWAP>(wr, xr, acc);
+    return mma_odd<2, SWAP>(wr, xr, acc);
+}
 typedef short s16x4 __attribute__((ext_vector_type(4)));
 __device__ __forceinline__ f4 mma16(u32x2 a, u32x2 b, f4 acc) {
     return __builtin_amdgcn_mfma_f32_16x16x16bf16_1k(__builtin_bit_cast(s16x4, a), __builtin_bit_cast(s16x4, b), acc, 0, 0, 0);
diff --git a/vittracker_amd/csrc/vt_blocks.h b/vittracker_amd/csrc/vt_blocks.h
--- a/vittracker_amd/csrc/vt_blocks.h
+++ b/vittracker_amd/csrc/vt_blocks.h
@@ -160,6 +160,9 @@
                                                          unsigned* __restrict__ vlscr) {
     static_assert(NW * TPW >= NT, "tiles must be covered");
     constexpr bool BF3L = BF3 && WLDS, BF3G = BF3 && !WLDS;
+    constexpr bool FOLD = BF3L;
+    using W2 = std::conditional_t<FOLD, vt3::odd_w, vt3::u32x2[3]>;
+    using X2 = std::conditional_t<FOLD, vt3::odd_x, vt3::u32x2[3]>;
     static_assert(!BF3L || (BAL && 2 * NT * NC >= W3_FC2_TILES - WBUF_TILES), "BF3 with staging: written for the balanced frame form; fc2's third output tile is staged in the K / V area");
     static_assert(!BAL || (WLDS && TPW == 1 && NW == 2 * (NT - 1)), "balanced variant: NT-1 owners + NT-1 guests");
     static_assert(!A3 || BF3, "A3: written for the three-piece forms");
@@ -233,7 +236,7 @@
         }
     }
     f4 x4s[NC];
-    f4 (&x4)[NC] = (BAL && !BF3) ? x[0] : x4s;
+    f4 (&x4)[NC] = BAL ? x[0] : x4s;
     if constexpr (BAL) {
         if (w >= NOWN) {
             const float* src = tokens + ((size_t)b * L + 16 * GT + tok) * C + 4 * q;
@@ -273,12 +276,34 @@
         const auto Wa3h = BF3L ? lds_lane_base<u32x2>(Wa, 192u * 16u + 8u * lane3) : nullptr;
         const auto Wb3 = BF3L ? lds_lane_base<u32x4>(Wb, 16u * lane3) : nullptr;
         const auto Wk3 = BF3L ? lds_lane_base<u32x4>(Kimg, 16u * lane3) : nullptr;
-        auto w1_load3 = [&](int t, u32x4 (&a0)[3], u32x2 (&a2)[3]) {
-#pragma unroll
-            for (int pc = 0; pc < 3; ++pc) {
-                a0[pc] = Wa3[t * W3_FC1_OT16 + pc * 64];
-                a2[pc] = Wa3h[t * W3_FC1_OT16 * 2 + pc * 64];
-            }
+        auto again = [](auto p) {
+            unsigned a = (unsigned)(uintptr_t)p;
+            asm volatile("" : "+v"(a));
+            return (decltype(p))(uintptr_t)a;
+        };
+        auto twin = [&](auto& p2, auto p) {
+            if constexpr (FOLD) p2 = again(p);
+        };
+        auto Wa3h2 = Wa3h;
+        auto ld_w2 = [&](W2& a2, lds_cptr<u32x2> p, lds_cptr<u32x2> p2, int idx) {
+            if constexpr (FOLD) a2 = vt3::ld_odd_w(p, p2, idx);
+            else {
+#pragma unroll
+                for (int pc = 0; pc < 3; ++pc) a2[pc] = p[idx + pc * 64];
+            }
+        };
+        auto xrow = [&](const u32x2 (&hc)[3]) -> decltype(auto) {
+            if constexpr (FOLD) return vt3::make_odd_x(hc);
+            else return (hc);
+        };
+        auto wrow = [&](const u32x2 (&a2)[3]) -> decltype(auto) {
+            if constexpr (FOLD) return vt3::make_odd_w(a2);
+            else return (a2);
+        };
+        auto w1_load3 = [&](int t, u32x4 (&a0)[3], W2& a2) {
+#pragma unroll
+            for (int pc = 0; pc < 3; ++pc) a0[pc] = Wa3[t * W3_FC1_OT16 + pc * 64];
+            ld_w2(a2, Wa3h, Wa3h2, t * W3_FC1_OT16 * 2);
         };
         auto w2_load3 = [&](int p, u32x4 (&a)[NC][3]) {
 #pragma unroll
@@ -295,35 +320,50 @@
 #pragma unroll
             for (int pc = 0; pc < 3; ++pc) hb[pc] = u32x4{a[pc].x, a[pc].y, b2[pc].x, b2[pc].y};
         };
-        auto tile48 = [&](auto swap, const u32x4 (&a0)[3], const u32x2 (&a2)[3], const u32x4 (&hb)[3], const u32x2 (&hc)[3], f4 init) {
+        auto tile48 = [&](auto swap, const u32x4 (&a0)[3], const W2& a2, const u32x4 (&hb)[3], const X2& hc, f4 init) {
             constexpr bool SWAP = decltype(swap)::value;
             constexpr int TW[6] = {2, 0, 1, 1, 0, 0}, TX[6] = {0, 2, 1, 0, 1, 0};
-            f4 accA = init, accB = splat4(0.f);
-#pragma unroll
-            for (int e = 0; e < 6; ++e) {
-                accB = SWAP ? vt3::mma16(hc[TX[e]], a2[TW[e]], accB) : vt3::mma16(a2[TW[e]], hc[TX[e]], accB);
-                accA = SWAP ? vt3::mma(hb[TX[e]], a0[TW[e]], accA) : vt3::mma(a0[TW[e]], hb[TX[e]], accA);
-            }
-            return accA + accB;
-        };
-        const auto Kp3 = A3 ? lds_lane_base<u32x4>(Kimg, 16u * lane3) : nullptr;
+            if constexpr (FOLD) {
+                f4 acc = init;
+#pragma unroll
+                for (int e = 0; e < 6; ++e) {
+                    acc = SWAP ? vt3::mma(hb[TX[e]], a0[TW[e]], acc) : vt3::mma(a0[TW[e]], hb[TX[e]], acc);
+                    if (e == 1) acc = vt3::mma_odd<0, SWAP>(a2, hc, acc);
+                    if (e == 3) acc = vt3::mma_odd<1, SWAP>(a2, hc, acc);
+                    if (e == 5) acc = vt3::mma_odd<2, SWAP>(a2, hc, acc);
+                }
+                return acc;
+            } else {
+                f4 accA = init, accB = splat4(0.f);
+#pragma unroll
+                for (int e = 0; e < 6; ++e) {
+                    accB = SWAP ? vt3::mma16(hc[TX[e]], a2[TW[e]], accB) : vt3::mma16(a2[TW[e]], hc[TX[e]], accB);
+                    accA = SWAP ? vt3::mma(hb[TX[e]], a0[TW[e]], accA) : vt3::mma(a0[TW[e]], hb[TX[e]], accA);
+                }
+                return accA + accB;
+            }
+        };
+        const auto Kp3 = VP3 ? Wk3 : A3 ? lds_lane_base<u32x4>(Kimg, 16u * lane3) : nullptr;
         const auto Kp3h = A3 ? lds_lane_base<u32x2>(Kimg, 192u * 16u + 8u * lane3) : nullptr;
-        const auto Vp3 = A3 ? lds_lane_base<u32x4>(Kimg + NT * KP_T16, 16u * lane3) : nullptr;
-        const auto Vp3h = A3 ? lds_lane_base<u32x2>(Kimg + NT * KP_T16, VP_PAIRS * 3 * 64 * 16u + 8u * lane3) : nullptr;
-        auto k_load3 = [&](int J, u32x4 (&a0)[3], u32x2 (&a2)[3]) {
-#pragma unroll
-            for (int pc = 0; pc < 3; ++pc) {
-                a0[pc] = Kp3[J * KP_T16 + pc * 64];
-                a2[pc] = Kp3h[J * KP_T16 * 2 + pc * 64];
-            }
-        };
-        auto wp_load3 = [&](int t, u32x4 (&a0)[3], u32x2 (&a2)[3]) {
+        const auto Vp3 = VP3 ? Kp3 + NT * KP_T16 : A3 ? lds_lane_base<u32x4>(Kimg + NT * KP_T16, 16u * lane3) : nullptr;
+        const auto Vp3h = VP3 ? Kp3h + (NT * KP_T16 + VP_PAIRS * 3 * 64 - 192) * 2
+                              : A3 ? lds_lane_base<u32x2>(Kimg + NT * KP_T16, VP_PAIRS * 3 * 64 * 16u + 8u * lane3) : nullptr;
+        auto Kp3h2 = Kp3h;
+        auto k_load3 = [&](int J, u32x4 (&a0)[3], W2& a2) {
+#pragma unroll
+            for (int pc = 0; pc < 3; ++pc) a0[pc] = Kp3[J * KP_T16 + pc * 64];
+            ld_w2(a2, Kp3h, Kp3h2, J * KP_T16 * 2);
+        };
+        lds_cptr<u32x2> Wp3h = nullptr, Wp3h2 = nullptr;
+        auto proj_bases = [&]() {
+            Wp3h = lds_lane_base<u32x2>(Wb, 192u * 16u + 8u * lane3);
+            twin(Wp3h2, Wp3h);
+        };
+        auto wp_load3 = [&](int t, u32x4 (&a0)[3], W2& a2) {
             if constexpr (BF3L) {
 #pragma unroll
-                for (int pc = 0; pc < 3; ++pc) {
-                    a0[pc] = Wb3[t * W3_FC1_OT16 + pc * 64];
-                    a2[pc] = reinterpret_cast<const u32x2*>(Wb)[(t * W3_FC1_OT16 + 192) * 2 + pc * 64 + lane3];
-                }
+                for (int pc = 0; pc < 3; ++pc) a0[pc] = Wb3[t * W3_FC1_OT16 + pc * 64];
+                ld_w2(a2, Wp3h, Wp3h2, t * W3_FC1_OT16 * 2);
             } else {
                 const u32x4* const Gp = reinterpret_cast<const u32x4*>(P3) + (W3_FC1_TILES + W3_FC2_TILES + W3_QKV_TILES) * 64;
 #pragma unroll
@@ -411,9 +451,11 @@
                     u32x4 hb[3];
                     u32x2 hc[3];
                     split_h3(h, hb, hc);
+                    const auto& hx = xrow(hc);
+                    twin(Wa3h2, Wa3h);
                     const u32x4* const Gq = reinterpret_cast<const u32x4*>(P3) + (W3_FC1_TILES + W3_FC2_TILES) * 64;
                     const u32x2* const Gqh = reinterpret_cast<const u32x2*>(Gq);
-                    auto wq_load3 = [&](int t, u32x4 (&a0)[3], u32x2 (&a2)[3]) {
+                    auto wq_load3 = [&](int t, u32x4 (&a0)[3], W2& a2) {
                         if constexpr (BF3L) w1_load3(t, a0, a2);
                         else {
 #pragma unroll
@@ -424,10 +466,9 @@
                         }
                     };
                     u32x4 a0[2][3];
-                    u32x2 a2[2][3];
+                    W2 a2[2];
                     auto bias_q = [&](int t) { return t < 2 * NC ? ld4(S + S_BQKV + 16 * t + 4 * q) : splat4(S[S_BQKV + 2 * C + 16 * (t % NC) + tok]); };
                     f4 bias[2];
-                    f4 kr[NC];
                     wq_load3(0, a0[0], a2[0]);
                     bias[0] = bias_q(0);
 #pragma unroll
@@ -439,15 +480,12 @@
                         const int ot = t % NC;
                         f4 r;
                         __builtin_amdgcn_sched_barrier(0);
-                        if (t < 2 * NC) r = tile48(std::false_type{}, a0[t & 1], a2[t & 1], hb, hc, bias[t & 1]);
-                        else r = tile48(std::true_type{}, a0[t & 1], a2[t & 1], hb, hc, bias[t & 1]);
+                        if (t < 2 * NC) r = tile48(std::false_type{}, a0[t & 1], a2[t & 1], hb, hx, bias[t & 1]);
+                        else r = tile48(std::true_type{}, a0[t & 1], a2[t & 1], hb, hx, bias[t & 1]);
                         if (t < NC) qr[i][ot] = r;
                         else if constexpr (A3) {
                             if (t < 2 * NC) {
-                                if constexpr (VP3) {
-                                    kr[ot] = r;
-                                    if (ot == NC - 1) store_k3(Kimg + T * KP_T16, kr);
-                                } else store_k3c(Kimg + T * KP_T16, ot, r);
+                                store_k3c(Kimg + T * KP_T16, ot, r);
                             } else if constexpr (VP3) store_v3(T, ot, r);
                             else if constexpr (VP2L) store_v2l(T, ot, r);
                             else Vo[(ot * NT + T) * 64 + lane] = to_opnd(r);
@@ -518,24 +556,30 @@
                     u32x4 hb[3];
                     u32x2 hc[3];
                     split_h3(h, hb, hc);
+                    const auto& hx = xrow(hc);
                     u32x4 a0[NC][3];
                     u32x2 a2[NC][3];
 #pragma unroll
-                    for (int j = 0; j < NC; ++j) w1_load3(NC * g + j, a0[j], a2[j]);
+                    for (int j = 0; j < NC; ++j)
+#pragma unroll
+                        for (int pc = 0; pc < 3; ++pc) {
+                            a0[j][pc] = Wa3[(NC * g + j) * W3_FC1_OT16 + pc * 64];
+                            a2[j][pc] = Wa3h[(NC * g + j) * W3_FC1_OT16 * 2 + pc * 64];
+                        }
                     if (g < 2) {
                         f4 bias[NC];
 #pragma unroll
                         for (int j = 0; j < NC; ++j) bias[j] = ld4(S + S_BQKV + 16 * (g * NC + j) + 4 * q);
                         __builtin_amdgcn_sched_barrier(0);
 #pragma unroll
-                        for (int j = 0; j < NC; ++j) r[j] = tile48(std::false_type{}, a0[j], a2[j], hb, hc, bias[j]);
+                        for (int j = 0; j < NC; ++j) r[j] = tile48(std::false_type{}, a0[j], wrow(a2[j]), hb, hx, bias[j]);
                     } else {
                         f4 bias[NC];
 #pragma unroll
                         for (int j = 0; j < NC; ++j) bias[j] = splat4(S[S_BQKV + 2 * C + 16 * j + tok]);
                         __builtin_amdgcn_sched_barrier(0);
 #pragma unroll
-                        for (int j = 0; j < NC; ++j) r[j] = tile48(std::true_type{}, a0[j], a2[j], hb, hc, bias[j]);
+                        for (int j = 0; j < NC; ++j) r[j] = tile48(std::true_type{}, a0[j], wrow(a2[j]), hb, hx, bias[j]);
                     }
                     if (zg_tile && zcache_mode == 1) {
                         f4* const zc = zc_guest();
@@ -623,19 +667,21 @@
                 u32x4 qb[3];
                 u32x2 qc[3];
                 split_h3(qr[i], qb, qc);
+                const auto& qx = xrow(qc);
+                twin(Kp3h2, Kp3h);
                 f4 s[NT];
                 float m0 = -3.0e38f, m1 = -3.0e38f;
                 {
                     constexpr int NB = VP3 ? 2 : 1;
                     u32x4 a0[NB][3];
-                    u32x2 a2[NB][3];
+                    W2 a2[NB];
                     if (NB == 2) k_load3(0, a0[0], a2[0]);
 #pragma unroll
                     for (int J = 0; J < NT; ++J) {
                         if (NB == 2 && J + 1 < NT) k_load3(J + 1, a0[(J + 1) % NB], a2[(J + 1) % NB]);
                         if (NB == 1) k_load3(J, a0[0], a2[0]);
                         __builtin_amdgcn_sched_barrier(0);
-                        s[J] = tile48(std::false_type{}, a0[J % NB], a2[J % NB], qb, qc, splat4(0.f));
+                        s[J] = tile48(std::false_type{}, a0[J % NB], a2[J % NB], qb, qx, splat4(0.f));
                         m0 = fmaxf(fmaxf(m0, s[J].x), s[J].y);
                         m1 = fmaxf(fmaxf(m1, s[J].z), s[J].w);
                     }
@@ -647,7 +693,7 @@
                 f4 o[NC];
                 constexpr int NWB = VP3 ? 2 : 1;
                 u32x4 wa0[NWB][3];
-                u32x2 wa2[NWB][3];
+                W2 wa2[NWB];
                 if constexpr (VP3) {
                     u32x4 pb[VP_PAIRS > 0 ? VP_PAIRS : 1][3];
                     u32x2 po[3], plo[3];
@@ -679,9 +725,9 @@
                     const f2 dd = d0 + d1;
                     const float rden = __builtin_amdgcn_rcpf(quad_sum(dd.x + dd.y));
                     fstamp();
-                    f4 oA[NC], oB[NC];
-#pragma unroll
-                    for (int t = 0; t < NC; ++t) oA[t] = oB[t] = splat4(0.f);
+                    f4 oA[NC];
+#pragma unroll
+                    for (int t = 0; t < NC; ++t) oA[t] = splat4(0.f);
                     u32x2 vh[NC][3];
                     if (NT & 1) {
 #pragma unroll
@@ -699,16 +745,20 @@
                         __builtin_amdgcn_sched_barrier(0);
                         if (pp + 1 < VP_PAIRS) v_load3(pp + 1);
                     }
+                    proj_bases();
                     wp_load3(0, wa0[0], wa2[0]);
                     if (NT & 1) {
                         __builtin_amdgcn_sched_barrier(0);
-#pragma unroll
-                        for (int e = 0; e < 6; ++e)
-#pragma unroll
-                            for (int t = 0; t < NC; ++t) oB[t] = vt3::mma16(vh[t][TW[e]], po[TX[e]], oB[t]);
-                    }
-#pragma unroll
-                    for (int t = 0; t < NC; ++t) o[t] = (oA[t] + oB[t]) * splat4(rden);
+                        const vt3::odd_x pr = vt3::make_odd_x(po);
+#pragma unroll
+                        for (int t = 0; t < NC; ++t) oA[t] = vt3::mma_odd<0>(vt3::make_odd_w(vh[t]), pr, oA[t]);
+#pragma unroll
+                        for (int t = 0; t < NC; ++t) oA[t] = vt3::mma_odd<1>(vt3::make_odd_w(vh[t]), pr, oA[t]);
+#pragma unroll
+                        for (int t = 0; t < NC; ++t) oA[t] = vt3::mma_odd<2>(vt3::make_odd_w(vh[t]), pr, oA[t]);
+                    }
+#pragma unroll
+                    for (int t = 0; t < NC; ++t) o[t] = oA[t] * splat4(rden);
                 } else if constexpr (VP2L) {
                     const auto Vp2 = lds_lane_base<u32x4>(Vimg, 16u * lane3);
                     const u32x4* const vlg = vl_blk + lane3;
@@ -785,12 +835,13 @@
                 u32x4 ob[3];
                 u32x2 oc[3];
                 split_h3(o, ob, oc);
+                const auto& ox = xrow(oc);
 #pragma unroll
                 for (int ot = 0; ot < NC; ++ot) {
                     if (NWB == 2 && ot + 1 < NC) wp_load3(ot + 1, wa0[(ot + 1) % NWB], wa2[(ot + 1) % NWB]);
                     if (NWB == 1) wp_load3(ot, wa0[0], wa2[0]);
                     __builtin_amdgcn_sched_barrier(0);
-                    x[i][ot] = tile48(std::false_type{}, wa0[ot % NWB], wa2[ot % NWB], ob, oc, x[i][ot] + ld4(S + S_BPROJ + 16 * ot + 4 * q));
+                    x[i][ot] = tile48(std::false_type{}, wa0[ot % NWB], wa2[ot % NWB], ob, ox, x[i][ot] + ld4(S + S_BPROJ + 16 * ot + 4 * q));
                     __builtin_amdgcn_sched_barrier(0);
                 }
             } else if (!A3 && VT_BLK_OWNERS && T - toff < NOWN && T != dbg_skip_tile && !(last_skip_z && 16 * T < len_z)) {
@@ -911,11 +962,11 @@
                 };
                 auto attn_part3 = [&](auto njc, int J0) {
                     constexpr int NJ = decltype(njc)::value;
-                    constexpr int TW[6] = {2, 0, 1, 1, 0, 0}, TX[6] = {0, 2, 1, 0, 1, 0};
                     u32x4 qb[3];
                     u32x2 qc[3];
                     u32x4 a0[NJ][3];
-                    u32x2 a2[NJ][3];
+                    W2 a2[NJ];
+                    twin(Kp3h2, Kp3h);
 #pragma unroll
                     for (int pc = 0; pc < 3; ++pc) {
                         qb[pc] = reinterpret_cast<const u32x4*>(Qg)[pc * 64 + lane3];
@@ -924,8 +975,7 @@
 #pragma unroll
                     for (int j = 0; j < NJ; ++j) k_load3(J0 + j, a0[j], a2[j]);
                     u32x2 vh[NJ][NC][3];
-#pragma unroll
-                    for (int j = 0; j < NJ; ++j) {
+                    auto vh_load = [&](int j) {
                         const int J = J0 + j;
                         const bool oddc = (NT & 1) && J == NT - 1;
 #pragma unroll
@@ -935,11 +985,15 @@
                             for (int pc = 0; pc < 3; ++pc)
                                 vh[j][t][pc] = oddc ? base[VP_PAIRS * 3 * 64 * 2 + pc * 64 + lane3] : base[(((J >> 1) * 3 + pc) * 64 + lane3) * 2 + (J & 1)];
                         }
-                    }
+                    };
+                    vh_load(0);
                     __builtin_amdgcn_sched_barrier(0);
                     f4 sc[NJ];
 #pragma unroll
-                    for (int j = 0; j < NJ; ++j) sc[j] = tile48(std::false_type{}, a0[j], a2[j], qb, qc, splat4(0.f));
+                    for (int j = 0; j < NJ; ++j) sc[j] = tile48(std::false_type{}, a0[j], a2[j], qb, xrow(qc), splat4(0.f));
+                    __builtin_amdgcn_sched_barrier(0);
+#pragma unroll
+                    for (int j = 1; j < NJ; ++j) vh_load(j);
                     float m0 = -3.0e38f, m1 = -3.0e38f;
 #pragma unroll
                     for (int j = 0; j < NJ; ++j) {
@@ -967,11 +1021,15 @@
 #pragma unroll
                     for (int t = 0; t < NC; ++t) o[t] = splat4(0.f);
 #pragma unroll
-                    for (int j = 0; j < NJ; ++j)
-#pragma unroll
-                        for (int e = 0; e < 6; ++e)
-#pragma unroll
-                            for (int t = 0; t < NC; ++t) o[t] = vt3::mma16(vh[j][t][TW[e]], pp[j][TX[e]], o[t]);
+                    for (int j = 0; j < NJ; ++j) {
+                        const vt3::odd_x pr = vt3::make_odd_x(pp[j]);
+#pragma unroll
+                        for (int t = 0; t < NC; ++t) o[t] = vt3::mma_odd<0>(vt3::make_odd_w(vh[j][t]), pr, o[t]);
+#pragma unroll
+                        for (int t = 0; t < NC; ++t) o[t] = vt3::mma_odd<1>(vt3::make_odd_w(vh[j][t]), pr, o[t]);
+#pragma unroll
+                        for (int t = 0; t < NC; ++t) o[t] = vt3::mma_odd<2>(vt3::make_odd_w(vh[j][t]), pr, o[t]);
+                    }
 #pragma unroll
                     for (int t = 0; t < NC; ++t) Pg[(g * NC + t) * 64 + lane] = o[t];
                     Mg[(g * 2 + 0) * 64 + lane] = m;
@@ -1013,10 +1071,12 @@
                     for (int t = 0; t < NC; ++t) o[t] = o[t] * splat4(rl);
                     if constexpr (A3) {
                         u32x4 ob[3], wa0[3];
-                        u32x2 oc[3], wa2[3];
+                        u32x2 oc[3];
+                        W2 wa2;
+                        proj_bases();
                         wp_load3(g, wa0, wa2);
                         split_h3(o, ob, oc);
-                        Dg[g * 64 + lane] = tile48(std::false_type{}, wa0, wa2, ob, oc, splat4(0.f));
+                        Dg[g * 64 + lane] = tile48(std::false_type{}, wa0, wa2, ob, xrow(oc), splat4(0.f));
                     } else {
                         f4 acc[1] = {splat4(0.f)};
                         gemm_stage<NC, 1, true, true>([&](int c, opnd (&a)[1]) { a[0] = w_proj(g * NC + c); },
@@ -1091,26 +1151,21 @@
             fstamp();
             fc2(hid[hi], 2, x[i]);
         };
-        auto fc1_terms3 = [&](auto nc, const u32x4 (*a0)[3], const u32x2 (*a2)[3], const u32x4 (&hb)[3], const u32x2 (&hc)[3], f4* acc) {
+        auto fc1_terms3 = [&](auto nc, const u32x4 (*a0)[3], const vt3::odd_w* a2, const u32x4 (&hb)[3], const u32x2 (&hc)[3], f4* acc) {
             constexpr int N = decltype(nc)::value;
             constexpr int TW[6] = {2, 0, 1, 1, 0, 0}, TX[6] = {0, 2, 1, 0, 1, 0};
-            f4 accB[N];
-#pragma unroll
-            for (int j = 0; j < N; ++j) accB[j] = splat4(0.f);
-#pragma unroll
-            for (int half = 0; half < 2; ++half)
-#pragma unroll
-                for (int k = 0; k < 2; ++k)
-#pragma unroll
-                    for (int t3 = 0; t3 < 3; ++t3)
-#pragma unroll
-                        for (int j = 0; j < N; ++j) {
-                            const int e = 3 * half + t3;
-                            if (k == 0) accB[j] = vt3::mma16(a2[j][TW[e]], hc[TX[e]], accB[j]);
-                            else acc[j] = vt3::mma(a0[j][TW[e]], hb[TX[e]], acc[j]);
-                        }
-#pragma unroll
-            for (int j = 0; j < N; ++j) acc[j] = acc[j] + accB[j];
+            const vt3::odd_x xr = vt3::make_odd_x(hc);
+#pragma unroll
+            for (int e = 0; e < 6; ++e) {
+#pragma unroll
+                for (int j = 0; j < N; ++j) acc[j] = vt3::mma(a0[j][TW[e]], hb[TX[e]], acc[j]);
+#pragma unroll
+                for (int j = 0; j < N; ++j) {
+                    if (e == 1) acc[j] = vt3::mma_odd<0>(a2[j], xr, acc[j]);
+                    if (e == 3) acc[j] = vt3::mma_odd<1>(a2[j], xr, acc[j]);
+                    if (e == 5) acc[j] = vt3::mma_odd<2>(a2[j], xr, acc[j]);
+                }
+            }
         };
         u32x4 hq[NHID][NH / 2][3];
         auto mlp_first3 = [&](int i, int hi) {
@@ -1121,11 +1176,18 @@
             u32x4 hb[3];
             u32x2 hc[3];
             split_h3(h, hb, hc);
+            const vt3::odd_x hx = vt3::make_odd_x(hc);
+            twin(Wa3h2, Wa3h);
             fstamp();
             constexpr int TW[6] = {2, 0, 1, 1, 0, 0}, TX[6] = {0, 2, 1, 0, 1, 0};
             u32x4 a0[2][3];
-            u32x2 a2[2][3];
-            w1_load3(0, a0[0], a2[0]);
+            vt3::odd_w a2[2];
+            auto w1_ld = [&](int t, u32x4 (&a)[3], vt3::odd_w& ao) {
+#pragma unroll
+                for (int pc = 0; pc < 3; ++pc) a[pc] = Wa3[t * W3_FC1_OT16 + pc * 64];
+                ao = vt3::ld_odd_w(Wa3h, Wa3h2, t * W3_FC1_OT16 * 2);
+            };
+            w1_ld(0, a0[0], a2[0]);
             f4 bias1[2];
             bias1[0] = ld4(S + S_B1 + 4 * q);
             f4 prev = splat4(0.f);
@@ -1208,11 +1270,11 @@
 #pragma unroll
             for (int t = 0; t <= NH; ++t) {
                 if (t == 4 || t == 8) fstamp();
-                f4 accA = splat4(0.f), accB = splat4(0.f);
+                f4 accA = splat4(0.f);
                 if (t < NH) {
                     accA = bias1[t & 1];
                     if (t + 1 < NH) {
-                        w1_load3(t + 1, a0[(t + 1) & 1], a2[(t + 1) & 1]);
+                        w1_ld(t + 1, a0[(t + 1) & 1], a2[(t + 1) & 1]);
                         bias1[(t + 1) & 1] = ld4(S + S_B1 + 16 * (t + 1) + 4 * q);
                     }
                 }
@@ -1220,8 +1282,10 @@
 #pragma unroll
                 for (int e = 0; e < 6; ++e) {
                     if (t < NH) {
-                        accB = vt3::mma16(a2[t & 1][TW[e]], hc[TX[e]], accB);
                         accA = vt3::mma(a0[t & 1][TW[e]], hb[TX[e]], accA);
+                        if (e == 1) accA = vt3::mma_odd<0>(a2[t & 1], hx, accA);
+                        if (e == 3) accA = vt3::mma_odd<1>(a2[t & 1], hx, accA);
+                        if (e == 5) accA = vt3::mma_odd<2>(a2[t & 1], hx, accA);
                     }
                     if (t > 0) {
                         if (e < 5) gstage(e);
@@ -1229,7 +1293,7 @@
                     }
                     __builtin_amdgcn_sched_barrier(0);
                 }
-                prev = accA + accB;
+                prev = accA;
             }
         };
         auto mlp_second3 = [&](int i, int hi) {
@@ -1265,8 +1329,9 @@
                 u32x4 hb[3];
                 u32x2 hc[3];
                 split_h3(h, hb, hc);
+                twin(Wa3h2, Wa3h);
                 u32x4 a0[NC][3];
-                u32x2 a2[NC][3];
+                W2 a2[NC];
 #pragma unroll
                 for (int j = 0; j < NC; ++j) w1_load3(NC * g + j, a0[j], a2[j]);
                 f4 acc[NC];
@@ -1297,37 +1362,23 @@
                     bh[pc] = odd ? gq[0][pc] : gq[2][pc];
                 }
                 u32x4 af[NC][3];
-                u32x2 ah[NC][3];
+                vt3::odd_w ah[NC];
                 w2_load3(p_full, af);
                 {
                     const unsigned hoff = 16u * lane3 + (odd ? 8u : 0u) + (unsigned)p_half * (3u * 64u * 16u);
                     const auto Wb3h = lds_lane_base<u32x2>(Wb, hoff);
                     const auto Wk3h = lds_lane_base<u32x2>(Kimg, hoff);
+                    const auto Wb3h2 = again(Wb3h);
+                    const auto Wk3h2 = again(Wk3h);
 #pragma unroll
                     for (int ot = 0; ot < NC; ++ot)
-#pragma unroll
-                        for (int pc = 0; pc < 3; ++pc)
-                            ah[ot][pc] = ot < 2 ? Wb3h[((ot * (NH / 2)) * 3 + pc) * 64 * 2] : Wk3h[pc * 64 * 2];
-                }
-                f4 part[NC], partB[NC];
-#pragma unroll
-                for (int ot = 0; ot < NC; ++ot) part[ot] = partB[ot] = splat4(0.f);
+                        ah[ot] = ot < 2 ? vt3::ld_odd_w(Wb3h, Wb3h2, (ot * (NH / 2)) * 3 * 64 * 2, 128) : vt3::ld_odd_w(Wk3h, Wk3h2, 0, 128);
+                }
+                f4 part[NC];
+#pragma unroll
+                for (int ot = 0; ot < NC; ++ot) part[ot] = splat4(0.f);
                 __builtin_amdgcn_sched_barrier(0);
-                constexpr int TW[6] = {2, 0, 1, 1, 0, 0}, TX[6] = {0, 2, 1, 0, 1, 0};
-#pragma unroll
-                for (int half = 0; half < 2; ++half)
-#pragma unroll
-                    for (int k = 0; k < 2; ++k)
-#pragma unroll
-                        for (int t3 = 0; t3 < 3; ++t3)
-#pragma unroll
-                            for (int ot = 0; ot < NC; ++ot) {
-                                const int e = 3 * half + t3;
-                                if (k == 0) partB[ot] = vt3::mma16(ah[ot][TW[e]], bh[TX[e]], partB[ot]);
-                                else part[ot] = vt3::mma(af[ot][TW[e]], bf[TX[e]], part[ot]);
-                            }
-#pragma unroll
-                for (int ot = 0; ot < NC; ++ot) part[ot] = part[ot] + partB[ot];
+                fc1_terms3(std::integral_constant<int, NC>{}, af, ah, bf, bh, part);
 #pragma unroll
                 for (int ot = 0; ot < NC; ++ot) Pg2[(g * NC + ot) * 64 + lane] = part[ot];
             }
@@ -1391,7 +1442,7 @@
                     const u32x4* const G1 = reinterpret_cast<const u32x4*>(P3);
                     const u32x2* const G1h = reinterpret_cast<const u32x2*>(P3);
                     const u32x4* const G2 = G1 + W3_FC1_TILES * 64;
-                    auto g1_load3 = [&](int t, u32x4 (&a0)[3], u32x2 (&a2)[3]) {
+                    auto g1_load3 = [&](int t, u32x4 (&a0)[3], W2& a2) {
 #pragma unroll
                         for (int pc = 0; pc < 3; ++pc) {
                             a0[pc] = G1[t * W3_FC1_OT16 + pc * 64 + lane3];
@@ -1403,10 +1454,12 @@
                     u32x4 hb[3];
                     u32x2 hc[3];
                     split_h3(h, hb, hc);
+                    const auto& hx = xrow(hc);
+                    twin(Wa3h2, Wa3h);
                     u32x4 hq3[NH / 2][3];
                     {
                         u32x4 a0[2][3];
-                        u32x2 a2[2][3];
+                        W2 a2[2];
                         g1_load3(0, a0[0], a2[0]);
                         u32x2 pl[3];
 #pragma unroll
@@ -1414,7 +1467,7 @@
                             if (t + 1 < NH) g1_load3(t + 1, a0[(t + 1) & 1], a2[(t + 1) & 1]);
                             const f4 bias = ld4(S + S_B1 + 16 * t + 4 * q);
                             __builtin_amdgcn_sched_barrier(0);
-                            const f4 r = tile48(std::false_type{}, a0[t & 1], a2[t & 1], hb, hc, bias);
+                            const f4 r = tile48(std::false_type{}, a0[t & 1], a2[t & 1], hb, hx, bias);
                             u32x2 pc3[3];
                             vt3::split3(gelu4(r), pc3[0], pc3[1], pc3[2]);
 #pragma unroll
```

New measurement: 3.413 million, median of 6. +4.8%, better.
